# Coder-Yu/SELFRec

Measured on NVIDIA H100. Metric: XSimGCL yelp2018 train steps/sec, higher is better.
Workload: dtype f32

## Files before the change

selfrec_b200/csrc/bpr.cu:

```cuda
#include "common.cuh"

namespace srb {

struct BprArgs {
  const float* emb;
  const float* l2_emb;
  int32_t n_users;
  const int32_t* u_idx;
  const int32_t* i_idx;
  const int32_t* j_idx;
  const int32_t* b_dev;
  int32_t b;
  float emb_scale;
  float reg;
  int32_t l2_terms;
  float l2_div;
  float grad_scale;
  float* losses;
  float* g_emb;
  float* g_l2;
  float* scratch;
};

template <int D>
__device__ __forceinline__ void load_row(const float* base, int row, int lane, float scale, float4 (&r)[(D + 127) / 128]) {
#pragma unroll
  for (int q = 0; q < (D + 127) / 128; ++q) {
    const int c = lane * 4 + q * 128;
    r[q] = (c < D) ? f4_scale(scale, ldg4(base + (size_t)row * D + c)) : f4_zero();
  }
}

template <int D>
__global__ void __launch_bounds__(256) bpr_reduce_kernel(const BprArgs a) {
  constexpr int Q = (D + 127) / 128;
  const int lane = threadIdx.x & 31;
  const int wib = threadIdx.x >> 5;
  const int t = blockIdx.x * (blockDim.x >> 5) + wib;
  const int b = a.b_dev ? min(*a.b_dev, a.b) : a.b;
  float bpr = 0.f, su = 0.f, sp = 0.f, sn = 0.f;
  if (t < b) {
    const int u = a.u_idx[t], p = a.n_users + a.i_idx[t], n = a.n_users + a.j_idx[t];
    float4 ru[Q], rp[Q], rn[Q];
    load_row<D>(a.emb, u, lane, a.emb_scale, ru);
    load_row<D>(a.emb, p, lane, a.emb_scale, rp);
    load_row<D>(a.emb, n, lane, a.emb_scale, rn);
    float pos = 0.f, neg = 0.f;
#pragma unroll
    for (int q = 0; q < Q; ++q) {
      pos += f4_dot(ru[q], rp[q]);
      neg += f4_dot(ru[q], rn[q]);
    }
    pos = warp_sum(pos);
    neg = warp_sum(neg);
    if (a.l2_emb != a.emb) {
      load_row<D>(a.l2_emb, u, lane, 1.f, ru);
      load_row<D>(a.l2_emb, p, lane, 1.f, rp);
      load_row<D>(a.l2_emb, n, lane, 1.f, rn);
    }
#pragma unroll
    for (int q = 0; q < Q; ++q) {
      su += f4_dot(ru[q], ru[q]);
      sp += f4_dot(rp[q], rp[q]);
      sn += f4_dot(rn[q], rn[q]);
    }
    su = warp_sum(su);
    sp = warp_sum(sp);
    sn = warp_sum(sn);
    const float x = pos - neg;
    const float sig = 1.f / (1.f + expf(-x));
    bpr = -logf(1e-5f + sig);
  }
  __shared__ float red[8][4];
  if (lane == 0) {
    red[wib][0] = bpr;
    red[wib][1] = su;
    red[wib][2] = sp;
    red[wib][3] = sn;
  }
  __syncthreads();
  if (threadIdx.x < 4) {
    float s = 0.f;
    for (int w = 0; w < (int)(blockDim.x >> 5); ++w) s += red[w][threadIdx.x];
    atomicAdd(a.scratch + threadIdx.x, s);
  }
}

template <int D>
__global__ void __launch_bounds__(256) bpr_grad_kernel(const BprArgs a) {
  constexpr int Q = (D + 127) / 128;
  const int lane = threadIdx.x & 31;
  const int t = blockIdx.x * (blockDim.x >> 5) + (threadIdx.x >> 5);
  const int b = a.b_dev ? min(*a.b_dev, a.b) : a.b;
  const float fb = (float)b;
  const float nu = sqrtf(a.scratch[1]), np = sqrtf(a.scratch[2]), nn = sqrtf(a.scratch[3]);
  if (blockIdx.x == 0 && threadIdx.x == 0) {
    a.losses[0] = (b > 0) ? a.scratch[0] / fb : 0.f;
    float l2 = nu + np + (a.l2_terms >= 3 ? nn : 0.f);
    a.losses[1] = (b > 0) ? a.reg * (l2 / fb) / a.l2_div : 0.f;
  }
  if (t >= b) return;
  const int u = a.u_idx[t], p = a.n_users + a.i_idx[t], n = a.n_users + a.j_idx[t];
  float4 ru[Q], rp[Q], rn[Q];
  load_row<D>(a.emb, u, lane, a.emb_scale, ru);
  load_row<D>(a.emb, p, lane, a.emb_scale, rp);
  load_row<D>(a.emb, n, lane, a.emb_scale, rn);
  float pos = 0.f, neg = 0.f;
#pragma unroll
  for (int q = 0; q < Q; ++q) {
    pos += f4_dot(ru[q], rp[q]);
    neg += f4_dot(ru[q], rn[q]);
  }
  pos = warp_sum(pos);
  neg = warp_sum(neg);
  const float x = pos - neg;
  const float sig = 1.f / (1.f + expf(-x));
  const float c = a.grad_scale * (-(sig * (1.f - sig)) / (1e-5f + sig)) / fb;
  const float k2 = a.grad_scale * a.reg / (fb * a.l2_div);
  const float ku = nu > 0.f ? k2 / nu : 0.f;
  const float kp = np > 0.f ? k2 / np : 0.f;
  const float kn = (a.l2_terms >= 3 && nn > 0.f) ? k2 / nn : 0.f;
  const bool l2_sep = (a.g_l2 != nullptr);
  float4 lu[Q], lp[Q], ln[Q];
  if (a.l2_emb != a.emb) {
    load_row<D>(a.l2_emb, u, lane, 1.f, lu);
    load_row<D>(a.l2_emb, p, lane, 1.f, lp);
    load_row<D>(a.l2_emb, n, lane, 1.f, ln);
  } else {
#pragma unroll
    for (int q = 0; q < Q; ++q) lu[q] = ru[q], lp[q] = rp[q], ln[q] = rn[q];
  }
  const size_t plane = (size_t)a.b * D;
#pragma unroll
  for (int q = 0; q < Q; ++q) {
    const int col = lane * 4 + q * 128;
    if (col >= D) continue;
    float4 gu = make_float4(c * (rp[q].x - rn[q].x), c * (rp[q].y - rn[q].y), c * (rp[q].z - rn[q].z), c * (rp[q].w - rn[q].w));
    float4 gp = f4_scale(c, ru[q]);
    float4 gn = f4_scale(-c, ru[q]);
    const float4 l2u = f4_scale(ku, lu[q]), l2p = f4_scale(kp, lp[q]), l2n = f4_scale(kn, ln[q]);
    const size_t o = (size_t)t * D + col;
    if (l2_sep) {
      st4(a.g_l2 + o, l2u);
      st4(a.g_l2 + plane + o, l2p);
      st4(a.g_l2 + 2 * plane + o, l2n);
    } else {
      gu = f4_add(gu, l2u);
      gp = f4_add(gp, l2p);
      gn = f4_add(gn, l2n);
    }
    st4(a.g_emb + o, gu);
    st4(a.g_emb + plane + o, gp);
    st4(a.g_emb + 2 * plane + o, gn);
  }
}

template <int D>
__global__ void __launch_bounds__(256) scatter_add_rows_kernel(float* dst, const ScatterSegs segs) {
  const ScatterSeg& sg = segs.s[blockIdx.y];
  const int lane = threadIdx.x & 31;
  const int r = blockIdx.x * (blockDim.x >> 5) + (threadIdx.x >> 5);
  const int nn = sg.n_dev ? min(*sg.n_dev, sg.n) : sg.n;
  if (r >= nn) return;
  int row = sg.rows[r] + sg.row_off;
  if (sg.row_hi > sg.row_lo) {
    if (row < sg.row_lo || row >= sg.row_hi) return;
    row -= sg.row_lo;
  } else if (sg.mod > 0) {
    if (row % sg.mod != sg.rem) return;
    row /= sg.mod;
  }
  for (int c = lane * 4; c < D; c += 128) {
    const float4 v = f4_scale(sg.scale, ldg4(sg.src + (size_t)r * D + c));
    atomicAdd(reinterpret_cast<float4*>(dst + (size_t)row * D + c), v);
  }
}

int scatter_segments(float* dst, int d, const ScatterSegs& segs, cudaStream_t st) {
  if (segs.count == 0) return SRB_OK;
  int max_n = 0;
  for (int q = 0; q < segs.count; ++q) max_n = segs.s[q].n > max_n ? segs.s[q].n : max_n;
  if (max_n == 0) return SRB_OK;
  dim3 grid((max_n + 7) / 8, segs.count);
  switch (d) {
    case 32: scatter_add_rows_kernel<32><<<grid, 256, 0, st>>>(dst, segs); break;
    case 64: scatter_add_rows_kernel<64><<<grid, 256, 0, st>>>(dst, segs); break;
    case 128: scatter_add_rows_kernel<128><<<grid, 256, 0, st>>>(dst, segs); break;
    default: set_error("scatter: unsupported d=%d (32, 64, 128)", d); return SRB_ERR_ARG;
  }
  return post_launch("scatter_add_rows_kernel");
}

struct L2Args {
  int n_terms;
  const float* x[4];
  float* g[4];
  long long n[4];
  int rows[4];
};

__global__ void __launch_bounds__(256) l2_sumsq_kernel(const L2Args a, float* sumsq) {
  const int t = blockIdx.y;
  const long long n = a.n[t];
  float acc = 0.f;
  for (long long i = (long long)blockIdx.x * blockDim.x + threadIdx.x; i < n; i += (long long)gridDim.x * blockDim.x) {
    const float v = a.x[t][i];
    acc = fmaf(v, v, acc);
  }
  acc = warp_sum(acc);
  __shared__ float red[8];
  if ((threadIdx.x & 31) == 0) red[threadIdx.x >> 5] = acc;
  __syncthreads();
  if (threadIdx.x == 0) {
    float s = 0.f;
    for (int w = 0; w < (int)(blockDim.x >> 5); ++w) s += red[w];
    atomicAdd(sumsq + t, s);
  }
}

__global__ void l2_loss_kernel(const L2Args a, const float* sumsq, float reg, float* loss) {
  float l = 0.f;
  for (int t = 0; t < a.n_terms; ++t) l += sqrtf(sumsq[t]) / (float)a.rows[t];
  *loss = l * reg;
}

__global__ void __launch_bounds__(256) l2_grad_kernel(const L2Args a, const float* sumsq, float reg, const float* gout) {
  const int t = blockIdx.y;
  const long long n = a.n[t];
  const float nrm = sqrtf(sumsq[t]);
  const float k = (nrm > 0.f) ? (*gout) * reg / ((float)a.rows[t] * nrm) : 0.f;
  for (long long i = (long long)blockIdx.x * blockDim.x + threadIdx.x; i < n; i += (long long)gridDim.x * blockDim.x)
    a.g[t][i] = k * a.x[t][i];
}

__global__ void adam_prepare_kernel(int32_t* step, float* scalars, double lr, double b1, double b2) {
  const int t = *step + 1;
  *step = t;
  const double bc1 = 1.0 - pow(b1, (double)t);
  const double bc2 = 1.0 - pow(b2, (double)t);
  scalars[0] = (float)(lr / bc1);
  scalars[1] = (float)sqrt(bc2);
}

__global__ void __launch_bounds__(256) adam_step_kernel(float* __restrict__ p, float* __restrict__ m, float* __restrict__ v,
                                                        const float* __restrict__ g, long long n4, long long n,
                                                        const float* __restrict__ scal, float w1, float b2, float w2, float eps) {
  const float step_size = scal[0], bc2_sqrt = scal[1];
  const long long stride = (long long)gridDim.x * blockDim.x;
  for (long long i = (long long)blockIdx.x * blockDim.x + threadIdx.x; i < n4; i += stride) {
    float4 pp = reinterpret_cast<float4*>(p)[i], mm = reinterpret_cast<float4*>(m)[i], vv = reinterpret_cast<float4*>(v)[i];
    const float4 gg = reinterpret_cast<const float4*>(g)[i];
#define SRB_ADAM1(F)                          \
  mm.F = mm.F + w1 * (gg.F - mm.F);           \
  vv.F = vv.F * b2;                           \
  vv.F = vv.F + (w2 * gg.F) * gg.F;           \
  pp.F = pp.F - step_size * (mm.F / (sqrtf(vv.F) / bc2_sqrt + eps));
    SRB_ADAM1(x) SRB_ADAM1(y) SRB_ADAM1(z) SRB_ADAM1(w)
#undef SRB_ADAM1
    reinterpret_cast<float4*>(p)[i] = pp;
    reinterpret_cast<float4*>(m)[i] = mm;
    reinterpret_cast<float4*>(v)[i] = vv;
  }
  for (long long i = n4 * 4 + (long long)blockIdx.x * blockDim.x + threadIdx.x; i < n; i += stride) {
    float mm = m[i], vv = v[i];
    const float gg = g[i];
    mm = mm + w1 * (gg - mm);
    vv = vv * b2;
    vv = vv + (w2 * gg) * gg;
    p[i] = p[i] - step_size * (mm / (sqrtf(vv) / bc2_sqrt + eps));
    m[i] = mm;
    v[i] = vv;
  }
}

}

extern "C" int srb_bpr_l2_fwd_bwd(const srb_bpr_desc* d, void* stream) {
  SRB_REQUIRE(d != nullptr, "bpr: null desc");
  SRB_REQUIRE(d->emb && d->u_idx && d->i_idx && d->j_idx && d->losses && d->g_emb && d->scratch, "bpr: null pointer");
  SRB_REQUIRE(d->l2_terms == 2 || d->l2_terms == 3, "bpr: l2_terms must be 2 or 3");
  SRB_REQUIRE(d->b >= 0, "bpr: negative batch");
  SRB_REQUIRE(d->l2_div > 0.f, "bpr: l2_div must be positive");
  srb::BprArgs a;
  a.emb = d->emb;
  a.l2_emb = d->l2_emb ? d->l2_emb : d->emb;
  SRB_REQUIRE(a.l2_emb == a.emb || d->g_l2, "bpr: a separate l2 table needs g_l2");
  a.n_users = d->n_users;
  a.u_idx = d->u_idx;
  a.i_idx = d->i_idx;
  a.j_idx = d->j_idx;
  a.b_dev = d->b_dev;
  a.b = d->b;
  a.emb_scale = d->emb_scale;
  a.reg = d->reg;
  a.l2_terms = d->l2_terms;
  a.l2_div = d->l2_div;
  a.grad_scale = d->grad_scale;
  a.losses = d->losses;
  a.g_emb = d->g_emb;
  a.g_l2 = d->g_l2;
  a.scratch = d->scratch;
  cudaStream_t st = (cudaStream_t)stream;
  SRB_TRY(srb::check_cuda(cudaMemsetAsync(d->scratch, 0, 8 * sizeof(float), st), "bpr memset"));
  const int blocks = d->b > 0 ? (d->b + 7) / 8 : 1;
  switch (d->d) {
#define SRB_CASE(DD)                                               \
  case DD:                                                         \
    srb::bpr_reduce_kernel<DD><<<blocks, 256, 0, st>>>(a);         \
    SRB_TRY(srb::post_launch("bpr_reduce_kernel"));                \
    srb::bpr_grad_kernel<DD><<<blocks, 256, 0, st>>>(a);           \
    return srb::post_launch("bpr_grad_kernel");
    SRB_CASE(32)
    SRB_CASE(64)
    SRB_CASE(128)
#undef SRB_CASE
    default: srb::set_error("bpr: unsupported d=%d (32, 64, 128)", d->d); return SRB_ERR_ARG;
  }
}

extern "C" int srb_scatter_add_rows(float* dst, int32_t d, const float* src, const int32_t* rows, int32_t n,
                                    const int32_t* n_dev, int32_t row_off, float scale, void* stream) {
  SRB_REQUIRE(dst && src && rows, "scatter: null pointer");
  SRB_REQUIRE(n >= 0, "scatter: negative n");
  srb::ScatterSegs segs;
  segs.count = 1;
  segs.s[0] = {src, rows, n_dev, n, row_off, scale, 0, 0};
  return srb::scatter_segments(dst, d, segs, (cudaStream_t)stream);
}

extern "C" int srb_scatter_add_segments(float* dst, int32_t d, int32_t n_segs, const srb_scatter_seg* in, void* stream) {
  SRB_REQUIRE(dst && in, "scatter: null pointer");
  SRB_REQUIRE(n_segs >= 0 && n_segs <= 8, "scatter: 0..8 segments per launch");
  srb::ScatterSegs segs;
  segs.count = n_segs;
  for (int q = 0; q < n_segs; ++q) {
    SRB_REQUIRE(in[q].src && in[q].rows && in[q].n >= 0, "scatter: bad segment %d", q);
    segs.s[q] = {in[q].src, in[q].rows, in[q].n_dev, in[q].n, in[q].row_off, in[q].scale, 0, 0};
  }
  return srb::scatter_segments(dst, d, segs, (cudaStream_t)stream);
}

extern "C" int srb_adam_prepare(int32_t* step_dev, float* scalars_dev, double lr, double beta1, double beta2, void* stream) {
  SRB_REQUIRE(step_dev && scalars_dev, "adam_prepare: null pointer");
  srb::adam_prepare_kernel<<<1, 1, 0, (cudaStream_t)stream>>>(step_dev, scalars_dev, lr, beta1, beta2);
  return srb::post_launch("adam_prepare_kernel");
}

extern "C" int srb_adam_step(float* p, float* m, float* v, const float* g, int64_t n, const float* scalars_dev, double beta1,
                             double beta2, float eps, void* stream) {
  SRB_REQUIRE(p && m && v && g && scalars_dev, "adam_step: null pointer");
  SRB_REQUIRE(n >= 0, "adam_step: negative n");
  if (n == 0) return SRB_OK;
  const long long n4 = (((uintptr_t)p | (uintptr_t)m | (uintptr_t)v | (uintptr_t)g) & 15) ? 0 : n / 4;
  long long blocks = (n4 + 255) / 256;
  const long long cap = (long long)srb::sm_count() * 8;
  if (blocks > cap) blocks = cap;
  if (blocks < 1) blocks = 1;
  srb::adam_step_kernel<<<(int)blocks, 256, 0, (cudaStream_t)stream>>>(p, m, v, g, n4, n, scalars_dev, (float)(1.0 - beta1), (float)beta2,
                                                                        (float)(1.0 - beta2), eps);
  return srb::post_launch("adam_step_kernel");
}

extern "C" int srb_l2_reg_fwd(int32_t n_terms, const float* const* x, const int64_t* n_elems, const int32_t* rows, float reg,
                              float* sumsq_dev, float* loss_dev, void* stream) {
  SRB_REQUIRE(n_terms >= 1 && n_terms <= 4, "l2_reg: 1..4 terms");
  SRB_REQUIRE(x && n_elems && rows && sumsq_dev && loss_dev, "l2_reg: null pointer");
  srb::L2Args a = {};
  a.n_terms = n_terms;
  long long mx = 1;
  for (int t = 0; t < n_terms; ++t) {
    SRB_REQUIRE(x[t] && rows[t] > 0 && n_elems[t] >= 0, "l2_reg: bad term %d", t);
    a.x[t] = x[t];
    a.n[t] = n_elems[t];
    a.rows[t] = rows[t];
    if (n_elems[t] > mx) mx = n_elems[t];
  }
  cudaStream_t st = (cudaStream_t)stream;
  SRB_TRY(srb::check_cuda(cudaMemsetAsync(sumsq_dev, 0, 4 * sizeof(float), st), "l2 memset"));
  long long bx = (mx + 255) / 256;
  if (bx > 1024) bx = 1024;
  srb::l2_sumsq_kernel<<<dim3((unsigned)bx, n_terms), 256, 0, st>>>(a, sumsq_dev);
  SRB_TRY(srb::post_launch("l2_sumsq_kernel"));
  srb::l2_loss_kernel<<<1, 1, 0, st>>>(a, sumsq_dev, reg, loss_dev);
  return srb::post_launch("l2_loss_kernel");
}

extern "C" int srb_l2_reg_bwd(int32_t n_terms, const float* const* x, float* const* g, const int64_t* n_elems,
                              const int32_t* rows, float reg, const float* sumsq_dev, const float* gout_dev, void* stream) {
  SRB_REQUIRE(n_terms >= 1 && n_terms <= 4, "l2_reg: 1..4 terms");
  SRB_REQUIRE(x && g && n_elems && rows && sumsq_dev && gout_dev, "l2_reg: null pointer");
  srb::L2Args a = {};
  a.n_terms = n_terms;
  long long mx = 1;
  for (int t = 0; t < n_terms; ++t) {
    SRB_REQUIRE(x[t] && g[t] && rows[t] > 0, "l2_reg: bad term %d", t);
    a.x[t] = x[t];
    a.g[t] = g[t];
    a.n[t] = n_elems[t];
    a.rows[t] = rows[t];
    if (n_elems[t] > mx) mx = n_elems[t];
  }
  long long bx = (mx + 255) / 256;
  if (bx > 1024) bx = 1024;
  srb::l2_grad_kernel<<<dim3((unsigned)bx, n_terms), 256, 0, (cudaStream_t)stream>>>(a, sumsq_dev, reg, gout_dev);
  return srb::post_launch("l2_grad_kernel");
}
```

selfrec_b200/csrc/common.cuh:

```cuda
#pragma once
#include <cuda_runtime.h>
#include <stdint.h>
#include <stdio.h>
#include <atomic>
#include "selfrec_b200.h"

#define SRB_FULL_MASK 0xffffffffu

namespace srb {

void set_error(const char* fmt, ...);
extern std::atomic<long long> g_launches;

inline int check_cuda(cudaError_t e, const char* what) {
  if (e != cudaSuccess) {
    set_error("%s: %s", what, cudaGetErrorString(e));
    return SRB_ERR_CUDA;
  }
  return SRB_OK;
}

inline int post_launch(const char* what) {
  g_launches.fetch_add(1, std::memory_order_relaxed);
  return check_cuda(cudaPeekAtLastError(), what);
}

#define SRB_REQUIRE(cond, ...)            \
  do {                                    \
    if (!(cond)) {                        \
      srb::set_error(__VA_ARGS__);        \
      return SRB_ERR_ARG;                 \
    }                                     \
  } while (0)

#define SRB_TRY(expr)                     \
  do {                                    \
    int _rc = (expr);                     \
    if (_rc != SRB_OK) return _rc;        \
  } while (0)

int sm_count();
long long l2_bytes();

struct ScatterSeg {
  const float* src;
  const int32_t* rows;
  const int32_t* n_dev;
  int32_t n;
  int32_t row_off;
  float scale;
  int32_t row_lo, row_hi;
  int32_t mod, rem;
};
struct ScatterSegs {
  int count;
  ScatterSeg s[8];
};
int scatter_segments(float* dst, int d, const ScatterSegs& segs, cudaStream_t st);

__device__ __forceinline__ float warp_sum(float v) {
#pragma unroll
  for (int o = 16; o > 0; o >>= 1) v += __shfl_xor_sync(SRB_FULL_MASK, v, o);
  return v;
}

__device__ __forceinline__ float4 ldg4(const float* p) {
  return __ldg(reinterpret_cast<const float4*>(p));
}

__device__ __forceinline__ void st4(float* p, const float4& v) {
  *reinterpret_cast<float4*>(p) = v;
}

__device__ __forceinline__ float4 f4_zero() { return make_float4(0.f, 0.f, 0.f, 0.f); }

__device__ __forceinline__ float4 f4_fma(float a, const float4& x, const float4& acc) {
  return make_float4(fmaf(a, x.x, acc.x), fmaf(a, x.y, acc.y), fmaf(a, x.z, acc.z),
                     fmaf(a, x.w, acc.w));
}

__device__ __forceinline__ float4 f4_add(const float4& a, const float4& b) {
  return make_float4(a.x + b.x, a.y + b.y, a.z + b.z, a.w + b.w);
}

__device__ __forceinline__ float4 f4_scale(float s, const float4& a) {
  return make_float4(s * a.x, s * a.y, s * a.z, s * a.w);
}

__device__ __forceinline__ float f4_dot(const float4& a, const float4& b) {
  return fmaf(a.w, b.w, fmaf(a.z, b.z, fmaf(a.y, b.y, a.x * b.x)));
}

__device__ __forceinline__ float sgnf(float x) {
  return (x > 0.f) ? 1.f : ((x < 0.f) ? -1.f : 0.f);
}

__device__ __forceinline__ uint4 philox4x32_10(uint4 ctr, uint2 key) {
  const uint32_t M0 = 0xD2511F53u, M1 = 0xCD9E8D57u, W0 = 0x9E3779B9u, W1 = 0xBB67AE85u;
#pragma unroll
  for (int r = 0; r < 10; ++r) {
    uint32_t hi0 = __umulhi(M0, ctr.x), lo0 = M0 * ctr.x;
    uint32_t hi1 = __umulhi(M1, ctr.z), lo1 = M1 * ctr.z;
    ctr = make_uint4(hi1 ^ ctr.y ^ key.x, lo1, hi0 ^ ctr.w ^ key.y, lo0);
    key.x += W0;
    key.y += W1;
  }
  return ctr;
}

__device__ __forceinline__ float u32_to_unit(uint32_t x) {
  return (float)(x >> 8) * (1.0f / 16777216.0f);
}

}
```

selfrec_b200/csrc/engine.cu:

```cuda
#include <mutex>
#include "common.cuh"

namespace srb {

struct Ws {
  float* final_;
  float* cl;
  float* v2;
  float* work0;
  float* work1;
  float* acc0;
  float* acc1;
  float* gd;
  float* rsum;
  float* g_emb;
  float* g_l2;
  float* g_nce;
  float* bpr_scratch;
  float* bpr_losses;
  float* nce_losses;
  int32_t* idx_cat;
  int32_t* n_cat;
  int32_t* batch_rows;
  int32_t* n_hub;
  uint32_t* row_mask;
  int32_t* hub_first;
  int32_t* hub_work;
  float* hub_part;
  int32_t hub_cap;
  void* nce_ws;
  int64_t nce_ws_bytes;
};

static int64_t al(int64_t x) { return (x + 255) / 256 * 256; }

static int64_t carve(const srb_step_desc* s, Ws* w, char* base) {
  const int64_t N = (int64_t)s->n_users + s->n_items, d = s->d, B = s->batch_cap;
  const int64_t nd = al(N * d * 4);
  int64_t off = 0;
  auto take = [&](int64_t bytes) {
    char* p = base ? base + off : nullptr;
    off += al(bytes);
    return p;
  };
  const bool graph = s->model != SRB_MODEL_MF;
  const bool two_views = s->model == SRB_MODEL_SIMGCL || s->model == SRB_MODEL_SGL;
  const bool has_cl = s->model == SRB_MODEL_XSIMGCL || two_views;
  float* f_final = (float*)take(graph ? nd : 0);
  float* f_cl = (float*)take(has_cl ? nd : 0);
  float* f_v2 = (float*)take(two_views ? nd : 0);
  float* f_w0 = (float*)take(graph ? nd : 0);
  float* f_w1 = (float*)take(graph ? nd : 0);
  float* f_a0 = (float*)take(nd);
  float* f_a1 = (float*)take(graph ? nd : 0);
  float* f_gd = (float*)take(graph ? nd : 0);
  float* f_rsum = (float*)take(graph ? nd : 0);
  float* f_gemb = (float*)take(3 * B * d * 4);
  float* f_gl2 = (float*)take(3 * B * d * 4);
  float* f_gnce = (float*)take(has_cl ? 4 * 2 * B * d * 4 : 0);
  float* f_bs = (float*)take(8 * 4);
  float* f_bl = (float*)take(2 * 4);
  float* f_nl = (float*)take(4 * 4);
  int32_t* i_cat = (int32_t*)take(2 * B * 4);
  int32_t* i_ncat = (int32_t*)take(4);
  int32_t* i_brows = (int32_t*)take(4 * 3 * B * 4);
  int32_t* i_nhub = (int32_t*)take(graph ? 32 + ((N + 31) / 32) * 4 : 32);
  uint32_t* u_mask = (uint32_t*)(i_nhub + 8);
  const int64_t hub_cap = graph ? s->adj.hub.n_work : 0;
  int32_t* i_hfirst = (int32_t*)take(hub_cap ? 3 * B * 4 : 0);
  int32_t* i_hwork = (int32_t*)take(hub_cap * 2 * 4);
  float* f_hpart = (float*)take(hub_cap * d * 4);
  const int64_t nws = has_cl ? srb_infonce_workspace_bytes((int32_t)(2 * B), (int32_t)d, 2) : 0;
  void* v_nws = take(nws);
  if (w) {
    w->final_ = f_final;
    w->cl = f_cl;
    w->v2 = f_v2;
    w->work0 = f_w0;
    w->work1 = f_w1;
    w->acc0 = f_a0;
    w->acc1 = f_a1;
    w->gd = f_gd;
    w->rsum = f_rsum;
    w->g_emb = f_gemb;
    w->g_l2 = f_gl2;
    w->g_nce = f_gnce;
    w->bpr_scratch = f_bs;
    w->bpr_losses = f_bl;
    w->nce_losses = f_nl;
    w->idx_cat = i_cat;
    w->n_cat = i_ncat;
    w->batch_rows = i_brows;
    w->n_hub = i_nhub;
    w->row_mask = u_mask;
    w->hub_first = i_hfirst;
    w->hub_work = i_hwork;
    w->hub_part = f_hpart;
    w->hub_cap = (int32_t)hub_cap;
    w->nce_ws = v_nws;
    w->nce_ws_bytes = nws;
  }
  return off;
}

__global__ void build_cat_idx_kernel(const int32_t* batch, int cap, int n_users, int32_t* idx_cat, int32_t* n_cat) {
  const int nu = min(batch[1], cap), ni = min(batch[2], cap);
  const int32_t* uu = batch + SRB_BATCH_HEADER + 3 * cap;
  const int32_t* ui = uu + cap;
  for (int t = blockIdx.x * blockDim.x + threadIdx.x; t < nu + ni; t += gridDim.x * blockDim.x)
    idx_cat[t] = (t < nu) ? uu[t] : n_users + ui[t - nu];
  if (blockIdx.x == 0 && threadIdx.x == 0) *n_cat = nu + ni;
}

__global__ void __launch_bounds__(256) build_batch_rows_kernel(const int32_t* batch, int cap, int n_users, const int32_t* rowptr,
                                                               int row_begin, int n_local, int32_t* rows, int32_t* counters,
                                                               uint32_t* row_mask, int32_t* hub_first, int32_t* hub_work,
                                                               int hub_cap) {
  const int t = blockIdx.x * blockDim.x + threadIdx.x;
  const int b = min(batch[0], cap);
  const int sec = t / cap, k = t % cap;
  if (sec >= 3 || k >= b) return;
  const int32_t* u = batch + SRB_BATCH_HEADER;
  const int grow = (sec == 0) ? u[k] : n_users + u[sec * cap + k];
  const uint32_t bit = 1u << (grow & 31);
  if (atomicOr(row_mask + (grow >> 5), bit) & bit) return;
  const int row = grow - row_begin;
  if (row < 0 || row >= n_local) return;
  const int deg = rowptr[row + 1] - rowptr[row];
  const int cls = (hub_first && deg >= SRB_HUB_MIN_NNZ) ? 0 : (deg >= 128 ? 1 : 2);
  const unsigned mine = __match_any_sync(__activemask(), cls);
  const int lane = threadIdx.x & 31;
  const int leader = __ffs(mine) - 1;
  int base = 0;
  if (lane == leader) base = atomicAdd(counters + cls, __popc(mine));
  base = __shfl_sync(mine, base, leader);
  const int slot = base + __popc(mine & ((1u << lane) - 1));
  rows[cls * 3 * cap + slot] = row;
  if (cls == 0) {
    const int nch = (deg + SRB_HUB_CHUNK - 1) / SRB_HUB_CHUNK;
    const int first = atomicAdd(counters + 4, nch);
    hub_first[slot] = first;
    for (int c = 0; c < nch && first + c < hub_cap; ++c) {
      hub_work[2 * (first + c)] = row;
      hub_work[2 * (first + c) + 1] = c;
    }
  }
}

__global__ void finalize_losses_kernel(const float* bpr_losses, const float* nce_losses, int n_nce, float cl_rate, float* out) {
  float cl = 0.f;
  for (int q = 0; q < n_nce; ++q) cl += nce_losses[q];
  cl *= cl_rate;
  out[0] = bpr_losses[0];
  out[1] = bpr_losses[1];
  out[2] = cl;
  out[3] = bpr_losses[0] + bpr_losses[1] + cl;
}

struct Chain {
  const srb_graph_csr* adj;
  ScatterSegs final_segs;
  ScatterSegs cl_segs;
  ScatterSegs ego_segs;
  int layer_cl;
  bool include_ego;
};

static int spmm_simple(const srb_step_desc* s, const srb_graph_csr* g, const float* x, float* y, const float* extra,
                       bool adam, cudaStream_t st, const uint32_t* col_mask = nullptr) {
  srb_spmm_desc p = {};
  p.col_mask = col_mask;
  p.rowptr = g->rowptr;
  p.colidx = g->colidx;
  p.vals = g->vals;
  p.row_order = g->row_order;
  p.n_long_rows = g->n_long_rows;
  p.n_vlong_rows = g->n_vlong_rows;
  p.hub = g->hub;
  p.n_rows = p.n_cols = s->n_users + s->n_items;
  p.d = s->d;
  p.X = x;
  p.Y = y;
  p.extra = extra;
  p.extra_scale = 1.f;
  if (adam) {
    p.adam_p = s->params;
    p.adam_m = s->adam_m;
    p.adam_v = s->adam_v;
    p.adam_scalars = s->scalars;
    p.beta1 = s->beta1;
    p.beta2 = s->beta2;
    p.adam_eps = s->adam_eps;
  }
  return srb_spmm_csr(&p, st);
}

struct ForkRes {
  cudaStream_t side;
  cudaEvent_t fork, join;
  bool ok;
};
static ForkRes* fork_res(const srb_step_desc* s, ForkRes* own) {
  if (s->fork_stream && s->fork_event && s->join_event) {
    own->side = (cudaStream_t)s->fork_stream;
    own->fork = (cudaEvent_t)s->fork_event;
    own->join = (cudaEvent_t)s->join_event;
    own->ok = true;
    return own;
  }
  static ForkRes res[64] = {};
  static std::mutex mu;
  int dev = 0;
  if (cudaGetDevice(&dev) != cudaSuccess || dev < 0 || dev >= 64) return nullptr;
  std::lock_guard<std::mutex> lock(mu);
  ForkRes& r = res[dev];
  if (!r.ok) {
    if (cudaStreamCreateWithFlags(&r.side, cudaStreamNonBlocking) != cudaSuccess) return nullptr;
    if (cudaEventCreateWithFlags(&r.fork, cudaEventDisableTiming) != cudaSuccess) return nullptr;
    if (cudaEventCreateWithFlags(&r.join, cudaEventDisableTiming) != cudaSuccess) return nullptr;
    r.ok = true;
  }
  return &r;
}

static ScatterSegs merged(const ScatterSegs& a, const ScatterSegs* b) {
  ScatterSegs m = a;
  if (b)
    for (int q = 0; q < b->count && m.count < 8; ++q) m.s[m.count++] = b->s[q];
  return m;
}

static int run_chain(const srb_step_desc* s, const Ws& w, const Chain& c, bool* gd_live, bool last, cudaStream_t st) {
  const int L = s->n_layers, d = s->d;
  const size_t bytes = (size_t)(s->n_users + s->n_items) * d * 4;
  SRB_TRY(check_cuda(cudaMemsetAsync(w.acc0, 0, bytes, st), "chain memset"));
  SRB_TRY(scatter_segments(w.acc0, d, merged(c.final_segs, c.layer_cl == L ? &c.cl_segs : nullptr), st));
  float* x = w.acc0;
  for (int k = L - 1; k >= 1; --k) {
    float* y = (x == w.acc0) ? w.acc1 : w.acc0;
    SRB_TRY(spmm_simple(s, c.adj, x, y, nullptr, false, st, k == L - 1 ? w.row_mask : nullptr));
    SRB_TRY(scatter_segments(y, d, merged(c.final_segs, c.layer_cl == k ? &c.cl_segs : nullptr), st));
    x = y;
  }
  const bool ego_add = (c.include_ego && c.final_segs.count) || c.ego_segs.count;
  if (ego_add && !*gd_live) {
    SRB_TRY(check_cuda(cudaMemsetAsync(w.gd, 0, bytes, st), "chain memset gd"));
    *gd_live = true;
  }
  if (ego_add) {
    if (c.include_ego) SRB_TRY(scatter_segments(w.gd, d, merged(c.final_segs, &c.ego_segs), st));
    else SRB_TRY(scatter_segments(w.gd, d, c.ego_segs, st));
  }
  const float* extra = *gd_live ? w.gd : nullptr;
  const uint32_t* mask = (L == 1) ? w.row_mask : nullptr;
  if (last) return spmm_simple(s, c.adj, x, nullptr, extra, true, st, mask);
  SRB_TRY(spmm_simple(s, c.adj, x, w.gd, extra, false, st, mask));
  *gd_live = true;
  return SRB_OK;
}

static ScatterSeg seg(const float* src, const int32_t* rows, const int32_t* n_dev, int n, int row_off, float scale) {
  ScatterSeg g = {src, rows, n_dev, n, row_off, scale, 0, 0};
  return g;
}

static int encoder(const srb_step_desc* s, const Ws& w, const srb_graph_csr* g, bool include_ego, int noise_mode, int view,
                   int layer_cl, float* final_out, float* cl_out, cudaStream_t st, const float* x1 = nullptr) {
  srb_encoder_desc e = {};
  e.rowptr = g->rowptr;
  e.colidx = g->colidx;
  e.vals = g->vals;
  e.row_order = g->row_order;
  e.n_long_rows = g->n_long_rows;
  e.n_vlong_rows = g->n_vlong_rows;
  e.hub = g->hub;
  e.n = s->n_users + s->n_items;
  e.d = s->d;
  e.n_layers = s->n_layers;
  e.include_ego = include_ego;
  e.layer_cl = layer_cl;
  e.noise_mode = noise_mode;
  if (noise_mode == 1) e.noise = s->noise + (size_t)view * s->n_layers * e.n * e.d;
  e.eps = s->eps;
  e.philox_seed = s->philox_seed;
  e.philox_offset = ((uint64_t)view << 32) | 0x10u;
  e.philox_step_dev = s->step_dev;
  e.E0 = s->params;
  if (cl_out && layer_cl == s->n_layers) {
    e.final_out = final_out;
  } else {
    e.last_rows = w.batch_rows;
    e.n_last_rows = 3 * s->batch_cap;
    e.last_rows_nv_dev = w.n_hub;
    e.last_rows_hub = srb_hub_split{0, w.hub_cap, w.hub_first, w.hub_work, w.hub_part};
    e.last_rows_out = final_out;
    e.final_out = w.rsum;
  }
  e.cl_out = cl_out;
  e.work0 = w.work0;
  e.work1 = w.work1;
  e.x1 = x1;
  return srb_encoder_forward(&e, st);
}

static int perturb_rows(const srb_step_desc* s, const float* x, float* out, int view, cudaStream_t st) {
  const size_t nd = (size_t)(s->n_users + s->n_items) * s->d;
  srb_spmm_desc p = {};
  p.rowptr = s->adj.rowptr;
  p.colidx = s->adj.colidx;
  p.vals = s->adj.vals;
  p.n_rows = p.n_cols = s->n_users + s->n_items;
  p.d = s->d;
  p.X = x;
  p.Y = out;
  p.extra_scale = 1.f;
  p.sum_scale = 1.f;
  p.noise_mode = s->noise_mode;
  if (s->noise_mode == 1) p.noise = s->noise + (size_t)view * s->n_layers * nd;
  p.eps = s->eps;
  p.philox_seed = s->philox_seed;
  p.philox_offset = ((uint64_t)view << 32) | 0x10u;
  p.philox_step_dev = s->step_dev;
  return srb_spmm_epilogue_rows(&p, st);
}

}

extern "C" int64_t srb_step_workspace_bytes(int32_t model, int32_t n, int32_t d, int32_t batch_cap, int32_t n_hub_work) {
  srb_step_desc s = {};
  s.adj.hub.n_work = n_hub_work > 0 ? n_hub_work : 0;
  s.model = model;
  s.n_users = n;
  s.n_items = 0;
  s.d = d;
  s.batch_cap = batch_cap;
  return srb::carve(&s, nullptr, nullptr);
}

extern "C" int srb_train_step(const srb_step_desc* s, void* stream) {
  using namespace srb;
  SRB_REQUIRE(s != nullptr, "step: null desc");
  SRB_REQUIRE(s->model >= SRB_MODEL_MF && s->model <= SRB_MODEL_SGL, "step: unknown model %d", s->model);
  SRB_REQUIRE(s->d == 32 || s->d == 64 || s->d == 128, "step: unsupported d=%d (32, 64, 128)", s->d);
  SRB_REQUIRE(s->n_users > 0 && s->n_items > 0 && s->batch_cap > 0, "step: bad sizes");
  SRB_REQUIRE(s->params && s->adam_m && s->adam_v && s->step_dev && s->scalars && s->losses && s->batch, "step: null pointer");
  SRB_REQUIRE(s->model == SRB_MODEL_MF || s->n_layers >= 1, "step: graph models need n_layers >= 1");
  SRB_REQUIRE(s->model == SRB_MODEL_MF || (s->adj.rowptr && s->adj.colidx && s->adj.vals), "step: null adjacency");
  const int N = s->n_users + s->n_items;
  const int64_t need = srb_step_workspace_bytes(s->model, N, s->d, s->batch_cap, s->model != SRB_MODEL_MF ? s->adj.hub.n_work : 0);
  SRB_REQUIRE(s->workspace && s->workspace_bytes >= need, "step: workspace too small (%lld < %lld)",
              (long long)s->workspace_bytes, (long long)need);
  SRB_REQUIRE(((uintptr_t)s->workspace & 255) == 0, "step: workspace must be 256-byte aligned");
  Ws w;
  carve(s, &w, (char*)s->workspace);
  cudaStream_t st = (cudaStream_t)stream;
  const int B = s->batch_cap, d = s->d, U = s->n_users, L = s->n_layers;
  const int32_t* hdr = s->batch;
  const int32_t* u_idx = s->batch + SRB_BATCH_HEADER;
  const int32_t* i_idx = u_idx + B;
  const int32_t* j_idx = i_idx + B;
  const int32_t* uq_u = j_idx + B;
  const int32_t* uq_i = uq_u + B;
  const int32_t* b_dev = hdr + 0;
  const int32_t* nu_dev = hdr + 1;
  const int32_t* ni_dev = hdr + 2;

  SRB_TRY(srb_adam_prepare(s->step_dev, s->scalars, s->lr, s->beta1, s->beta2, stream));

  if (s->model != SRB_MODEL_MF) {
    SRB_TRY(check_cuda(cudaMemsetAsync(w.n_hub, 0, 32 + (size_t)((U + s->n_items + 31) / 32) * 4, st), "row mask memset"));
    build_batch_rows_kernel<<<(3 * B + 255) / 256, 256, 0, st>>>(s->batch, B, U, s->adj.rowptr, 0, U + s->n_items, w.batch_rows, w.n_hub,
                                                                   w.row_mask, w.hub_cap ? w.hub_first : nullptr, w.hub_work, w.hub_cap);
    SRB_TRY(post_launch("build_batch_rows_kernel"));
  }
  const float* table = s->params;
  int n_nce = 0;
  switch (s->model) {
    case SRB_MODEL_MF: break;
    case SRB_MODEL_LIGHTGCN:
      SRB_TRY(encoder(s, w, &s->adj, true, 0, 0, 0, w.final_, nullptr, st));
      table = w.final_;
      break;
    case SRB_MODEL_XSIMGCL:
      SRB_REQUIRE(s->noise_mode == 1 || s->noise_mode == 2, "step: XSimGCL needs noise_mode 1 or 2");
      SRB_REQUIRE(s->noise_mode != 1 || s->noise, "step: noise tensor missing");
      SRB_TRY(encoder(s, w, &s->adj, false, s->noise_mode, 0, s->layer_cl, w.final_, w.cl, st));
      table = w.final_;
      break;
    case SRB_MODEL_SIMGCL:
      SRB_REQUIRE(s->noise_mode == 1 || s->noise_mode == 2, "step: SimGCL needs noise_mode 1 or 2");
      SRB_REQUIRE(s->noise_mode != 1 || s->noise, "step: noise tensor missing");
      if (L >= 2) {
        SRB_TRY(spmm_simple(s, &s->adj, s->params, w.acc0, nullptr, false, st));
        SRB_TRY(perturb_rows(s, w.acc0, w.acc1, 0, st));
        SRB_TRY(perturb_rows(s, w.acc0, w.gd, 1, st));
        SRB_TRY(encoder(s, w, &s->adj, false, 0, 0, 0, w.final_, nullptr, st, w.acc0));
        SRB_TRY(encoder(s, w, &s->adj, false, s->noise_mode, 0, 0, w.cl, nullptr, st, w.acc1));
        SRB_TRY(encoder(s, w, &s->adj, false, s->noise_mode, 1, 0, w.v2, nullptr, st, w.gd));
      } else {
        SRB_TRY(encoder(s, w, &s->adj, false, 0, 0, 0, w.final_, nullptr, st));
        SRB_TRY(encoder(s, w, &s->adj, false, s->noise_mode, 0, 0, w.cl, nullptr, st));
        SRB_TRY(encoder(s, w, &s->adj, false, s->noise_mode, 1, 0, w.v2, nullptr, st));
      }
      table = w.final_;
      break;
    case SRB_MODEL_SGL:
      SRB_REQUIRE(s->adj_view[0].rowptr && s->adj_view[1].rowptr, "step: SGL needs two view graphs");
      SRB_TRY(encoder(s, w, &s->adj, true, 0, 0, 0, w.final_, nullptr, st));
      SRB_TRY(encoder(s, w, &s->adj_view[0], true, 0, 0, 0, w.cl, nullptr, st));
      SRB_TRY(encoder(s, w, &s->adj_view[1], true, 0, 0, 0, w.v2, nullptr, st));
      table = w.final_;
      break;
  }

  ForkRes fk_own = {};
  ForkRes* fk = (s->model == SRB_MODEL_XSIMGCL || s->model == SRB_MODEL_SIMGCL || s->model == SRB_MODEL_SGL) ? fork_res(s, &fk_own) : nullptr;
  if (fk) {
    SRB_TRY(check_cuda(cudaEventRecord(fk->fork, st), "fork record"));
    SRB_TRY(check_cuda(cudaStreamWaitEvent(fk->side, fk->fork, 0), "fork wait"));
  }
  {
    srb_bpr_desc p = {};
    p.emb = table;
    p.l2_emb = (s->model == SRB_MODEL_LIGHTGCN) ? s->params : table;
    p.n_users = U;
    p.d = d;
    p.u_idx = u_idx;
    p.i_idx = i_idx;
    p.j_idx = j_idx;
    p.b_dev = b_dev;
    p.b = B;
    p.emb_scale = 1.f;
    p.reg = s->reg;
    p.l2_terms = (s->model == SRB_MODEL_SIMGCL || s->model == SRB_MODEL_XSIMGCL) ? 2 : 3;
    p.l2_div = s->l2_div;
    p.grad_scale = 1.f;
    p.losses = w.bpr_losses;
    p.g_emb = w.g_emb;
    p.g_l2 = (s->model == SRB_MODEL_LIGHTGCN) ? w.g_l2 : nullptr;
    p.scratch = w.bpr_scratch;
    SRB_TRY(srb_bpr_l2_fwd_bwd(&p, fk ? (void*)fk->side : stream));
    if (fk) SRB_TRY(check_cuda(cudaEventRecord(fk->join, fk->side), "join record"));
  }

  const size_t gn = (size_t)2 * B * d;
  float* g1a = w.g_nce;
  float* g2a = w.g_nce + gn;
  float* g1b = w.g_nce + 2 * gn;
  float* g2b = w.g_nce + 3 * gn;
  if (s->model == SRB_MODEL_XSIMGCL || s->model == SRB_MODEL_SIMGCL) {
    srb_infonce_desc q = {};
    q.n_problems = 2;
    q.d = d;
    q.b_cos = 1;
    q.temperature = s->tau;
    const float* t1 = (s->model == SRB_MODEL_XSIMGCL) ? w.final_ : w.cl;
    const float* t2 = (s->model == SRB_MODEL_XSIMGCL) ? w.cl : w.v2;
    q.prob[0] = {t1, t2, 0, 0, 1.f, 1.f, uq_u, nu_dev, B, s->cl_rate, g1a, g2a, w.nce_losses + 0};
    q.prob[1] = {t1, t2, U, U, 1.f, 1.f, uq_i, ni_dev, B, s->cl_rate, g1b, g2b, w.nce_losses + 1};
    q.workspace = w.nce_ws;
    q.workspace_bytes = w.nce_ws_bytes;
    SRB_TRY(srb_infonce_fwd_bwd(&q, stream));
    n_nce = 2;
  } else if (s->model == SRB_MODEL_SGL) {
    build_cat_idx_kernel<<<8, 256, 0, st>>>(s->batch, B, U, w.idx_cat, w.n_cat);
    SRB_TRY(post_launch("build_cat_idx_kernel"));
    srb_infonce_desc q = {};
    q.n_problems = 1;
    q.d = d;
    q.b_cos = 1;
    q.temperature = s->tau;
    q.prob[0] = {w.cl, w.v2, 0, 0, 1.f, 1.f, w.idx_cat, w.n_cat, 2 * B, s->cl_rate, g1a, g2a, w.nce_losses + 0};
    q.workspace = w.nce_ws;
    q.workspace_bytes = w.nce_ws_bytes;
    SRB_TRY(srb_infonce_fwd_bwd(&q, stream));
    n_nce = 1;
  }
  if (fk) SRB_TRY(check_cuda(cudaStreamWaitEvent(st, fk->join, 0), "join wait"));
  finalize_losses_kernel<<<1, 1, 0, st>>>(w.bpr_losses, w.nce_losses, n_nce, s->cl_rate, s->losses);
  SRB_TRY(post_launch("finalize_losses_kernel"));

  const size_t plane = (size_t)B * d;
  if (s->model == SRB_MODEL_MF) {
    const size_t bytes = (size_t)N * d * 4;
    SRB_TRY(check_cuda(cudaMemsetAsync(w.acc0, 0, bytes, st), "mf memset"));
    ScatterSegs sg;
    sg.count = 3;
    sg.s[0] = seg(w.g_emb, u_idx, b_dev, B, 0, 1.f);
    sg.s[1] = seg(w.g_emb + plane, i_idx, b_dev, B, U, 1.f);
    sg.s[2] = seg(w.g_emb + 2 * plane, j_idx, b_dev, B, U, 1.f);
    SRB_TRY(scatter_segments(w.acc0, d, sg, st));
    return srb_adam_step(s->params, s->adam_m, s->adam_v, w.acc0, (int64_t)N * d, s->scalars, s->beta1, s->beta2, s->adam_eps,
                         stream);
  }
  const float cm = 1.f / (float)((s->model == SRB_MODEL_LIGHTGCN || s->model == SRB_MODEL_SGL) ? L + 1 : L);
  bool gd_live = false;
  if (s->model == SRB_MODEL_SGL) {
    for (int v = 0; v < 2; ++v) {
      Chain c = {};
      c.adj = &s->adj_view[v];
      c.include_ego = true;
      c.final_segs.count = 1;
      c.final_segs.s[0] = seg(v == 0 ? g1a : g2a, w.idx_cat, w.n_cat, 2 * B, 0, cm);
      SRB_TRY(run_chain(s, w, c, &gd_live, false, st));
    }
  }
  Chain c = {};
  c.adj = &s->adj;
  c.include_ego = (s->model == SRB_MODEL_LIGHTGCN || s->model == SRB_MODEL_SGL);
  ScatterSegs& f = c.final_segs;
  f.count = 3;
  f.s[0] = seg(w.g_emb, u_idx, b_dev, B, 0, cm);
  f.s[1] = seg(w.g_emb + plane, i_idx, b_dev, B, U, cm);
  f.s[2] = seg(w.g_emb + 2 * plane, j_idx, b_dev, B, U, cm);
  if (s->model == SRB_MODEL_LIGHTGCN) {
    c.ego_segs.count = 3;
    c.ego_segs.s[0] = seg(w.g_l2, u_idx, b_dev, B, 0, 1.f);
    c.ego_segs.s[1] = seg(w.g_l2 + plane, i_idx, b_dev, B, U, 1.f);
    c.ego_segs.s[2] = seg(w.g_l2 + 2 * plane, j_idx, b_dev, B, U, 1.f);
  } else if (s->model == SRB_MODEL_XSIMGCL) {
    f.count = 5;
    f.s[3] = seg(g1a, uq_u, nu_dev, B, 0, cm);
    f.s[4] = seg(g1b, uq_i, ni_dev, B, U, cm);
    ScatterSegs& cs = (s->layer_cl >= 1 && s->layer_cl <= L) ? c.cl_segs : c.ego_segs;
    cs.count = 2;
    cs.s[0] = seg(g2a, uq_u, nu_dev, B, 0, 1.f);
    cs.s[1] = seg(g2b, uq_i, ni_dev, B, U, 1.f);
    c.layer_cl = (s->layer_cl >= 1 && s->layer_cl <= L) ? s->layer_cl : 0;
  } else if (s->model == SRB_MODEL_SIMGCL) {
    f.count = 7;
    f.s[3] = seg(g1a, uq_u, nu_dev, B, 0, cm);
    f.s[4] = seg(g1b, uq_i, ni_dev, B, U, cm);
    f.s[5] = seg(g2a, uq_u, nu_dev, B, 0, cm);
    f.s[6] = seg(g2b, uq_i, ni_dev, B, U, cm);
  }
  return run_chain(s, w, c, &gd_live, true, st);
}
```

selfrec_b200/csrc/infonce.cu:

```cuda
#include <stdlib.h>
#include "common.cuh"
#include "infonce_tc.cuh"

namespace srb {

constexpr int NCE_T = 64;
constexpr int NCE_MAX_SPLITS = 8;

struct NceProblem {
  const float* table1;
  const float* table2;
  int32_t row_off1, row_off2;
  float scale1, scale2;
  const int32_t* idx;
  const int32_t* n_dev;
  int32_t n;
  float weight;
  float* g1;
  float* g2;
  float* loss;
  float* V1;
  float* V2;
  float* V1T;
  float* V2T;
  float* inv1;
  float* inv2;
  float* diag;
  float* part_m;
  float* part_l;
  float* dV1;
  float* dV2;
  float* loss_acc;
  float* lse;
};

struct NceArgs {
  int32_t n_problems;
  int32_t np;
  int32_t splits;
  int32_t b_cos;
  float inv_tau;
  NceProblem p[4];
};

__device__ __forceinline__ float tf32_rna(float x) {
  uint32_t r;
  asm("cvt.rna.tf32.f32 %0, %1;" : "=r"(r) : "f"(x));
  return __uint_as_float(r);
}

__device__ __forceinline__ int nce_n(const NceProblem& p) { return p.n_dev ? min(*p.n_dev, p.n) : p.n; }

template <int D>
__global__ void __launch_bounds__(256) nce_prep_kernel(const NceArgs a) {
  const NceProblem& p = a.p[blockIdx.y];
  const int lane = threadIdx.x & 31;
  const int i = blockIdx.x * (blockDim.x >> 5) + (threadIdx.x >> 5);
  if (i >= a.np) return;
  const int n = nce_n(p);
  if (blockIdx.x == 0 && threadIdx.x == 0) *p.loss_acc = 0.f;
  constexpr int Q = (D + 127) / 128;
  float4 v1[Q], v2[Q];
  float s1 = 0.f, s2 = 0.f, s12 = 0.f;
  if (i < n) {
    const int r = p.idx[i];
#pragma unroll
    for (int q = 0; q < Q; ++q) {
      const int c = lane * 4 + q * 128;
      v1[q] = (c < D) ? f4_scale(p.scale1, ldg4(p.table1 + (size_t)(r + p.row_off1) * D + c)) : f4_zero();
      v2[q] = (c < D) ? f4_scale(p.scale2, ldg4(p.table2 + (size_t)(r + p.row_off2) * D + c)) : f4_zero();
      s1 += f4_dot(v1[q], v1[q]);
      s2 += f4_dot(v2[q], v2[q]);
    }
  } else {
#pragma unroll
    for (int q = 0; q < Q; ++q) v1[q] = f4_zero(), v2[q] = f4_zero();
  }
  s1 = warp_sum(s1);
  s2 = warp_sum(s2);
  float i1 = 1.f, i2 = 1.f;
  if (a.b_cos) {
    i1 = 1.f / fmaxf(sqrtf(s1), 1e-12f);
    i2 = 1.f / fmaxf(sqrtf(s2), 1e-12f);
  }
#pragma unroll
  for (int q = 0; q < Q; ++q) {
    const int c = lane * 4 + q * 128;
    if (a.b_cos) {
      const float n1 = fmaxf(sqrtf(s1), 1e-12f), n2 = fmaxf(sqrtf(s2), 1e-12f);
      v1[q] = make_float4(v1[q].x / n1, v1[q].y / n1, v1[q].z / n1, v1[q].w / n1);
      v2[q] = make_float4(v2[q].x / n2, v2[q].y / n2, v2[q].z / n2, v2[q].w / n2);
    }
    s12 += f4_dot(v1[q], v2[q]);
    if (c < D) {
      st4(p.V1 + (size_t)i * D + c, v1[q]);
      st4(p.V2 + (size_t)i * D + c, v2[q]);
      st4(p.dV1 + (size_t)i * D + c, f4_zero());
      st4(p.dV2 + (size_t)i * D + c, f4_zero());
      p.V1T[(size_t)(c + 0) * a.np + i] = v1[q].x;
      p.V1T[(size_t)(c + 1) * a.np + i] = v1[q].y;
      p.V1T[(size_t)(c + 2) * a.np + i] = v1[q].z;
      p.V1T[(size_t)(c + 3) * a.np + i] = v1[q].w;
      p.V2T[(size_t)(c + 0) * a.np + i] = v2[q].x;
      p.V2T[(size_t)(c + 1) * a.np + i] = v2[q].y;
      p.V2T[(size_t)(c + 2) * a.np + i] = v2[q].z;
      p.V2T[(size_t)(c + 3) * a.np + i] = v2[q].w;
    }
  }
  s12 = warp_sum(s12);
  if (lane == 0) {
    p.inv1[i] = i1;
    p.inv2[i] = i2;
    p.diag[i] = s12 * a.inv_tau;
  }
}

__global__ void __launch_bounds__(256) nce_prep_tc_kernel(const NceArgs a) {
  constexpr int D = 64;
  __shared__ float t1[32][D + 1], t2[32][D + 1];
  const NceProblem& p = a.p[blockIdx.y];
  const int lane = threadIdx.x & 31, warp = threadIdx.x >> 5;
  const int i0 = blockIdx.x * 32;
  const int n = nce_n(p);
  if (blockIdx.x == 0 && threadIdx.x == 0) *p.loss_acc = 0.f;
  const size_t nd = (size_t)a.np * D;
  float* hi = p.dV2 + nd;
  float* lo = hi + 4 * nd;
#pragma unroll 1
  for (int rr = 0; rr < 4; ++rr) {
    const int il = warp * 4 + rr, i = i0 + il;
    const int c = lane * 2;
    float2 v1 = make_float2(0.f, 0.f), v2 = make_float2(0.f, 0.f);
    if (i < n) {
      const int r = p.idx[i];
      v1 = *reinterpret_cast<const float2*>(p.table1 + (size_t)(r + p.row_off1) * D + c);
      v2 = *reinterpret_cast<const float2*>(p.table2 + (size_t)(r + p.row_off2) * D + c);
      v1.x *= p.scale1, v1.y *= p.scale1, v2.x *= p.scale2, v2.y *= p.scale2;
    }
    const float s1 = warp_sum(v1.x * v1.x + v1.y * v1.y);
    const float s2 = warp_sum(v2.x * v2.x + v2.y * v2.y);
    float i1 = 1.f, i2 = 1.f;
    if (a.b_cos) {
      const float n1 = fmaxf(sqrtf(s1), 1e-12f), n2 = fmaxf(sqrtf(s2), 1e-12f);
      i1 = 1.f / n1, i2 = 1.f / n2;
      v1.x /= n1, v1.y /= n1, v2.x /= n2, v2.y /= n2;
    }
    const float s12 = warp_sum(v1.x * v2.x + v1.y * v2.y);
    const size_t o = (size_t)i * D + c;
    *reinterpret_cast<float2*>(p.V1 + o) = v1;
    *reinterpret_cast<float2*>(p.V2 + o) = v2;
    *reinterpret_cast<float2*>(p.dV1 + o) = make_float2(0.f, 0.f);
    *reinterpret_cast<float2*>(p.dV2 + o) = make_float2(0.f, 0.f);
    const float2 h1 = make_float2(tf32_rna(v1.x), tf32_rna(v1.y)), h2 = make_float2(tf32_rna(v2.x), tf32_rna(v2.y));
    *reinterpret_cast<float2*>(hi + o) = h1;
    *reinterpret_cast<float2*>(hi + nd + o) = h2;
    *reinterpret_cast<float2*>(lo + o) = make_float2(v1.x - h1.x, v1.y - h1.y);
    *reinterpret_cast<float2*>(lo + nd + o) = make_float2(v2.x - h2.x, v2.y - h2.y);
    t1[il][c] = v1.x, t1[il][c + 1] = v1.y;
    t2[il][c] = v2.x, t2[il][c + 1] = v2.y;
    if (lane == 0) {
      p.inv1[i] = i1;
      p.inv2[i] = i2;
      p.diag[i] = s12 * a.inv_tau;
      p.part_l[i] = 0.f;
    }
  }
  __syncthreads();
  for (int e = threadIdx.x; e < D * 32; e += 256) {
    const int dc = e >> 5, il = e & 31;
    const size_t o = (size_t)dc * a.np + i0 + nce_tperm(il);
    const float x1 = t1[il][dc], x2 = t2[il][dc];
    const float g1 = tf32_rna(x1), g2 = tf32_rna(x2);
    hi[2 * nd + o] = g1;
    hi[3 * nd + o] = g2;
    lo[2 * nd + o] = x1 - g1;
    lo[3 * nd + o] = x2 - g2;
  }
}

template <int D>
__device__ __forceinline__ void load_kmajor(float (*dst)[NCE_T], const float* T, int np, int col0) {
  for (int e = threadIdx.x; e < D * (NCE_T / 4); e += blockDim.x) {
    const int k = e / (NCE_T / 4), c4 = e % (NCE_T / 4);
    *reinterpret_cast<float4*>(&dst[k][c4 * 4]) = *reinterpret_cast<const float4*>(T + (size_t)k * np + col0 + c4 * 4);
  }
}

template <int D>
__device__ __forceinline__ void load_rowmajor(float (*dst)[D], const float* V, int row0) {
  for (int e = threadIdx.x; e < NCE_T * (D / 4); e += blockDim.x) {
    const int r = e / (D / 4), c4 = e % (D / 4);
    *reinterpret_cast<float4*>(&dst[r][c4 * 4]) = *reinterpret_cast<const float4*>(V + (size_t)(row0 + r) * D + c4 * 4);
  }
}

template <int D>
__device__ __forceinline__ void s_tile(const float (*AsT)[NCE_T], const float (*BsT)[NCE_T], int ty, int tx, float (&s)[4][4]) {
#pragma unroll
  for (int r = 0; r < 4; ++r)
#pragma unroll
    for (int c = 0; c < 4; ++c) s[r][c] = 0.f;
#pragma unroll 8
  for (int k = 0; k < D; ++k) {
    const float4 av = *reinterpret_cast<const float4*>(&AsT[k][ty * 4]);
    const float4 bv = *reinterpret_cast<const float4*>(&BsT[k][tx * 4]);
    const float ar[4] = {av.x, av.y, av.z, av.w};
    const float bc[4] = {bv.x, bv.y, bv.z, bv.w};
#pragma unroll
    for (int r = 0; r < 4; ++r)
#pragma unroll
      for (int c = 0; c < 4; ++c) s[r][c] = fmaf(ar[r], bc[c], s[r][c]);
  }
}

template <int D>
struct NceLseSmem {
  float AsT[D][NCE_T];
  float BsT[D][NCE_T];
};

template <int D>
__global__ void __launch_bounds__(256) nce_lse_kernel(const NceArgs a) {
  extern __shared__ __align__(16) unsigned char smem_raw[];
  NceLseSmem<D>& sm = *reinterpret_cast<NceLseSmem<D>*>(smem_raw);
  const NceProblem& p = a.p[blockIdx.z];
  const int n = nce_n(p);
  const int i0 = blockIdx.x * NCE_T;
  if (i0 >= n) return;
  const int split = blockIdx.y;
  const int ty = threadIdx.x >> 4, tx = threadIdx.x & 15;
  load_kmajor<D>(sm.AsT, p.V1T, a.np, i0);
  float m[4], l[4];
#pragma unroll
  for (int r = 0; r < 4; ++r) m[r] = -INFINITY, l[r] = 0.f;
  const int ntiles = (n + NCE_T - 1) / NCE_T;
  const float L2E = 1.4426950408889634f;
  for (int jt = split; jt < ntiles; jt += a.splits) {
    const int j0 = jt * NCE_T;
    __syncthreads();
    load_kmajor<D>(sm.BsT, p.V2T, a.np, j0);
    __syncthreads();
    float s[4][4];
    s_tile<D>(sm.AsT, sm.BsT, ty, tx, s);
#pragma unroll
    for (int r = 0; r < 4; ++r) {
      float tm = -INFINITY;
#pragma unroll
      for (int c = 0; c < 4; ++c) {
        s[r][c] = (j0 + tx * 4 + c < n) ? s[r][c] * a.inv_tau : -INFINITY;
        tm = fmaxf(tm, s[r][c]);
      }
      const float mn = fmaxf(m[r], tm);
      if (mn > -INFINITY) {
        float acc = 0.f;
#pragma unroll
        for (int c = 0; c < 4; ++c) acc += exp2f((s[r][c] - mn) * L2E);
        l[r] = l[r] * exp2f((m[r] - mn) * L2E) + acc;
        m[r] = mn;
      }
    }
  }
#pragma unroll
  for (int r = 0; r < 4; ++r) {
#pragma unroll
    for (int o = 8; o > 0; o >>= 1) {
      const float mo = __shfl_xor_sync(SRB_FULL_MASK, m[r], o);
      const float lo = __shfl_xor_sync(SRB_FULL_MASK, l[r], o);
      const float mn = fmaxf(m[r], mo);
      if (mn > -INFINITY) {
        l[r] = l[r] * exp2f((m[r] - mn) * L2E) + lo * exp2f((mo - mn) * L2E);
        m[r] = mn;
      }
    }
    if (tx == 0) {
      const int i = i0 + ty * 4 + r;
      p.part_m[(size_t)split * a.np + i] = m[r];
      p.part_l[(size_t)split * a.np + i] = l[r];
    }
  }
}

template <int D>
struct NceGradSmem {
  float AsT[D][NCE_T];
  float BsT[D][NCE_T];
  float Ar[NCE_T][D];
  float Br[NCE_T][D];
  float Gs[NCE_T][NCE_T];
  float GsT[NCE_T][NCE_T];
  float lse[NCE_T];
  float red[8];
};

template <int D>
__global__ void __launch_bounds__(256) nce_grad_kernel(const NceArgs a) {
  constexpr int CW = D / 16;
  extern __shared__ __align__(16) unsigned char smem_raw[];
  NceGradSmem<D>& sm = *reinterpret_cast<NceGradSmem<D>*>(smem_raw);
  const NceProblem& p = a.p[blockIdx.z];
  const int n = nce_n(p);
  const int i0 = blockIdx.x * NCE_T;
  if (i0 >= n) return;
  const int split = blockIdx.y;
  const int ty = threadIdx.x >> 4, tx = threadIdx.x & 15;
  const float L2E = 1.4426950408889634f;
  load_kmajor<D>(sm.AsT, p.V1T, a.np, i0);
  load_rowmajor<D>(sm.Ar, p.V1, i0);
  if (threadIdx.x < NCE_T) {
    const int i = i0 + threadIdx.x;
    float M = -INFINITY;
    for (int s = 0; s < a.splits; ++s) M = fmaxf(M, p.part_m[(size_t)s * a.np + i]);
    float Lsum = 0.f;
    for (int s = 0; s < a.splits; ++s) {
      const float ms = p.part_m[(size_t)s * a.np + i];
      if (ms > -INFINITY) Lsum += p.part_l[(size_t)s * a.np + i] * exp2f((ms - M) * L2E);
    }
    const float lse = (i < n) ? M + logf(Lsum) : 0.f;
    sm.lse[threadIdx.x] = lse;
    float contrib = (split == 0 && i < n) ? lse - p.diag[i] : 0.f;
    contrib = warp_sum(contrib);
    if ((threadIdx.x & 31) == 0) sm.red[threadIdx.x >> 5] = contrib;
  }
  __syncthreads();
  if (threadIdx.x == 0 && split == 0) atomicAdd(p.loss_acc, sm.red[0] + sm.red[1]);
  const float gscale = p.weight * a.inv_tau / (float)n;
  float o1[4][CW];
#pragma unroll
  for (int r = 0; r < 4; ++r)
#pragma unroll
    for (int q = 0; q < CW; ++q) o1[r][q] = 0.f;
  const int ntiles = (n + NCE_T - 1) / NCE_T;
  for (int jt = split; jt < ntiles; jt += a.splits) {
    const int j0 = jt * NCE_T;
    __syncthreads();
    load_kmajor<D>(sm.BsT, p.V2T, a.np, j0);
    load_rowmajor<D>(sm.Br, p.V2, j0);
    __syncthreads();
    float s[4][4];
    s_tile<D>(sm.AsT, sm.BsT, ty, tx, s);
#pragma unroll
    for (int r = 0; r < 4; ++r) {
      const int i = i0 + ty * 4 + r;
      const float lse = sm.lse[ty * 4 + r];
#pragma unroll
      for (int c = 0; c < 4; ++c) {
        const int j = j0 + tx * 4 + c;
        float g = 0.f;
        if (i < n && j < n) {
          g = exp2f((s[r][c] * a.inv_tau - lse) * L2E);
          if (i == j) g -= 1.f;
          g *= gscale;
        }
        s[r][c] = g;
      }
      *reinterpret_cast<float4*>(&sm.Gs[ty * 4 + r][tx * 4]) = make_float4(s[r][0], s[r][1], s[r][2], s[r][3]);
    }
#pragma unroll
    for (int c = 0; c < 4; ++c) {
      const int jl = tx * 4 + c;
      *reinterpret_cast<float4*>(&sm.GsT[jl][((ty ^ (jl >> 2)) & 15) * 4]) = make_float4(s[0][c], s[1][c], s[2][c], s[3][c]);
    }
    __syncthreads();
#pragma unroll 4
    for (int j = 0; j < NCE_T; ++j) {
      const float4 av = *reinterpret_cast<const float4*>(&sm.GsT[j][((ty ^ (j >> 2)) & 15) * 4]);
      const float ar[4] = {av.x, av.y, av.z, av.w};
      float bq[CW];
#pragma unroll
      for (int q = 0; q < CW; ++q) bq[q] = sm.Br[j][tx * CW + q];
#pragma unroll
      for (int r = 0; r < 4; ++r)
#pragma unroll
        for (int q = 0; q < CW; ++q) o1[r][q] = fmaf(ar[r], bq[q], o1[r][q]);
    }
    float qv[4][CW];
#pragma unroll
    for (int r = 0; r < 4; ++r)
#pragma unroll
      for (int q = 0; q < CW; ++q) qv[r][q] = 0.f;
#pragma unroll 4
    for (int i = 0; i < NCE_T; ++i) {
      const float4 av = *reinterpret_cast<const float4*>(&sm.Gs[i][ty * 4]);
      const float ar[4] = {av.x, av.y, av.z, av.w};
      float bq[CW];
#pragma unroll
      for (int q = 0; q < CW; ++q) bq[q] = sm.Ar[i][tx * CW + q];
#pragma unroll
      for (int r = 0; r < 4; ++r)
#pragma unroll
        for (int q = 0; q < CW; ++q) qv[r][q] = fmaf(ar[r], bq[q], qv[r][q]);
    }
#pragma unroll
    for (int r = 0; r < 4; ++r) {
      const int j = j0 + ty * 4 + r;
      if (j < n) {
#pragma unroll
        for (int q = 0; q < CW; ++q) atomicAdd(p.dV2 + (size_t)j * D + tx * CW + q, qv[r][q]);
      }
    }
  }
#pragma unroll
  for (int r = 0; r < 4; ++r) {
    const int i = i0 + ty * 4 + r;
    if (i < n) {
#pragma unroll
      for (int q = 0; q < CW; ++q) atomicAdd(p.dV1 + (size_t)i * D + tx * CW + q, o1[r][q]);
    }
  }
}

template <int D>
__global__ void __launch_bounds__(256) nce_finish_kernel(const NceArgs a) {
  const NceProblem& p = a.p[blockIdx.y];
  const int lane = threadIdx.x & 31;
  const int i = blockIdx.x * (blockDim.x >> 5) + (threadIdx.x >> 5);
  const int n = nce_n(p);
  if (blockIdx.x == 0 && threadIdx.x == 0) *p.loss = (n > 0) ? *p.loss_acc / (float)n : 0.f;
  if (i >= n) return;
  constexpr int Q = (D + 127) / 128;
#pragma unroll 1
  for (int side = 0; side < 2; ++side) {
    const float* V = side ? p.V2 : p.V1;
    const float* dV = side ? p.dV2 : p.dV1;
    float* g = side ? p.g2 : p.g1;
    const float inv = side ? p.inv2[i] : p.inv1[i];
    float4 vh[Q], dv[Q];
    float dot = 0.f;
#pragma unroll
    for (int q = 0; q < Q; ++q) {
      const int c = lane * 4 + q * 128;
      vh[q] = (c < D) ? *reinterpret_cast<const float4*>(V + (size_t)i * D + c) : f4_zero();
      dv[q] = (c < D) ? *reinterpret_cast<const float4*>(dV + (size_t)i * D + c) : f4_zero();
      dot += f4_dot(vh[q], dv[q]);
    }
    dot = warp_sum(dot);
#pragma unroll
    for (int q = 0; q < Q; ++q) {
      const int c = lane * 4 + q * 128;
      if (c >= D) continue;
      float4 o = dv[q];
      if (a.b_cos) {
        o = make_float4((dv[q].x - vh[q].x * dot) * inv, (dv[q].y - vh[q].y * dot) * inv, (dv[q].z - vh[q].z * dot) * inv,
                        (dv[q].w - vh[q].w * dot) * inv);
      }
      st4(g + (size_t)i * D + c, o);
    }
  }
}

static inline int64_t align_up(int64_t x, int64_t a) { return (x + a - 1) / a * a; }
static inline int nce_np(int n) { return (int)align_up(n > 0 ? n : 1, 128); }

static int64_t nce_problem_floats(int np, int d) {
  return 14ll * np * d + 4ll * np + 2ll * NCE_MAX_SPLITS * np + 64;
}

__global__ void __launch_bounds__(256) nce_tc_finish_kernel(const NceArgs a) {
  constexpr int D = 64;
  const NceProblem& p = a.p[blockIdx.y];
  const int lane = threadIdx.x & 31;
  const int i = blockIdx.x * (blockDim.x >> 5) + (threadIdx.x >> 5);
  const int n = nce_n(p);
  if (blockIdx.x == 0 && threadIdx.x == 0) *p.loss = (n > 0) ? *p.loss_acc / (float)n : 0.f;
  if (i >= n) return;
  const float li = p.part_l[i];
  const float pii = expf(p.diag[i] - a.inv_tau) / li;
  const float gs = p.weight * a.inv_tau / (float)n;
  const float cd = (pii - 1.f) * gs;
  const float2 v1 = *reinterpret_cast<const float2*>(p.V1 + (size_t)i * D + lane * 2);
  const float2 v2 = *reinterpret_cast<const float2*>(p.V2 + (size_t)i * D + lane * 2);
#pragma unroll 1
  for (int side = 0; side < 2; ++side) {
    const float2 vh = side ? v2 : v1;
    const float2 vo = side ? v1 : v2;
    float2 dv = *reinterpret_cast<const float2*>((side ? p.dV2 : p.dV1) + (size_t)i * D + lane * 2);
    if (side == 0) dv.x *= gs / li, dv.y *= gs / li;
    dv.x = fmaf(cd, vo.x, dv.x);
    dv.y = fmaf(cd, vo.y, dv.y);
    const float dot = warp_sum(vh.x * dv.x + vh.y * dv.y);
    const float inv = side ? p.inv2[i] : p.inv1[i];
    float2 o = dv;
    if (a.b_cos) o = make_float2((dv.x - vh.x * dot) * inv, (dv.y - vh.y * dot) * inv);
    *reinterpret_cast<float2*>((side ? p.g2 : p.g1) + (size_t)i * D + lane * 2) = o;
  }
}

static int nce_impl() {
  static int impl = -1;
  if (impl < 0) {
    const char* e = getenv("SRB_NCE_IMPL");
    impl = e ? atoi(e) : 0;
  }
  return impl;
}

static int nce_launch_tc(const NceArgs& a, int n_problems, cudaStream_t st) {
  const int np = a.np;
  const int d = NT_D;
  {
    dim3 grid(np / 32, n_problems);
    nce_prep_tc_kernel<<<grid, 256, 0, st>>>(a);
    SRB_TRY(post_launch("nce_prep_tc_kernel"));
  }
  NtMaps maps;
  NtArgs t;
  t.np = np;
  t.inv_tau = a.inv_tau;
  const int row_blocks = np / NT_T;
  int splits = sm_count() / (row_blocks * n_problems);
  if (splits < 1) splits = 1;
  if (splits > NT_MAX_SPLITS) splits = NT_MAX_SPLITS;
  if (splits > row_blocks) splits = row_blocks;
  t.splits = splits;
  const long long nd = (long long)np * d;
  for (int q = 0; q < n_problems; ++q) {
    const NceProblem& p = a.p[q];
    float* hi = p.dV2 + nd;
    float* lo = hi + 4 * nd;
    for (int h = 0; h < 2; ++h) {
      float* r = h ? lo : hi;
      SRB_REQUIRE(make_tmap_f32_rows(&maps.v1r[q][h], r, (uint64_t)np, d, NT_T) == 0 &&
                      make_tmap_f32_rows(&maps.v2r[q][h], r + nd, (uint64_t)np, d, NT_T) == 0 &&
                      make_tmap_f32_rows(&maps.v1c[q][h], r, (uint64_t)np, d, NT_C) == 0 &&
                      make_tmap_f32_rows(&maps.v2c[q][h], r + nd, (uint64_t)np, d, NT_C) == 0 &&
                      make_tmap_f32_rows(&maps.v1t[q][h], r + 2 * nd, (uint64_t)d, (uint64_t)np, NT_D) == 0 &&
                      make_tmap_f32_rows(&maps.v2t[q][h], r + 3 * nd, (uint64_t)d, (uint64_t)np, NT_D) == 0,
                  "infonce: cuTensorMapEncodeTiled failed");
    }
    NtProblem& o = t.p[q];
    o.n = p.n;
    o.n_dev = p.n_dev;
    o.weight = p.weight;
    o.diag = p.diag;
    o.lsum = p.part_l;
    o.dV1 = p.dV1;
    o.dV2 = p.dV2;
    o.loss_acc = p.loss_acc;
  }
  for (int q = n_problems; q < 2; ++q) {
    for (int h = 0; h < 2; ++h) {
      maps.v1r[q][h] = maps.v1r[0][h];
      maps.v2r[q][h] = maps.v2r[0][h];
      maps.v1c[q][h] = maps.v1c[0][h];
      maps.v2c[q][h] = maps.v2c[0][h];
      maps.v1t[q][h] = maps.v1t[0][h];
      maps.v2t[q][h] = maps.v2t[0][h];
    }
    t.p[q] = t.p[0];
  }
  const size_t smem = NtSmem::total + 1024;
  static bool attr_done = false;
  if (!attr_done) {
    SRB_TRY(check_cuda(cudaFuncSetAttribute(nce_tc_kernel<1>, cudaFuncAttributeMaxDynamicSharedMemorySize, (int)smem), "nce tc attr"));
    SRB_TRY(check_cuda(cudaFuncSetAttribute(nce_tc_kernel<2>, cudaFuncAttributeMaxDynamicSharedMemorySize, (int)smem), "nce tc attr"));
    attr_done = true;
  }
  dim3 grid(row_blocks, splits, n_problems);
  nce_tc_kernel<1><<<grid, NT_THREADS, smem, st>>>(maps, t);
  SRB_TRY(post_launch("nce_tc_kernel<pass_a>"));
  nce_tc_kernel<2><<<grid, NT_THREADS, smem, st>>>(maps, t);
  SRB_TRY(post_launch("nce_tc_kernel<pass_b>"));
  {
    dim3 g2((np + 7) / 8, n_problems);
    nce_tc_finish_kernel<<<g2, 256, 0, st>>>(a);
    SRB_TRY(post_launch("nce_tc_finish_kernel"));
  }
  return SRB_OK;
}

template <int D>
static int nce_launch(const NceArgs& a, int n_problems, cudaStream_t st) {
  const int np = a.np;
  {
    dim3 grid((np + 7) / 8, n_problems);
    nce_prep_kernel<D><<<grid, 256, 0, st>>>(a);
    SRB_TRY(post_launch("nce_prep_kernel"));
  }
  {
    static bool attr_done = false;
    if (!attr_done) {
      SRB_TRY(check_cuda(cudaFuncSetAttribute(nce_lse_kernel<D>, cudaFuncAttributeMaxDynamicSharedMemorySize, (int)sizeof(NceLseSmem<D>)), "nce lse smem attr"));
      SRB_TRY(check_cuda(cudaFuncSetAttribute(nce_grad_kernel<D>, cudaFuncAttributeMaxDynamicSharedMemorySize, (int)sizeof(NceGradSmem<D>)), "nce grad smem attr"));
      attr_done = true;
    }
    dim3 grid(np / NCE_T, a.splits, n_problems);
    nce_lse_kernel<D><<<grid, 256, sizeof(NceLseSmem<D>), st>>>(a);
    SRB_TRY(post_launch("nce_lse_kernel"));
    nce_grad_kernel<D><<<grid, 256, sizeof(NceGradSmem<D>), st>>>(a);
    SRB_TRY(post_launch("nce_grad_kernel"));
  }
  {
    dim3 grid((np + 7) / 8, n_problems);
    nce_finish_kernel<D><<<grid, 256, 0, st>>>(a);
    SRB_TRY(post_launch("nce_finish_kernel"));
  }
  return SRB_OK;
}

}

extern "C" int64_t srb_infonce_workspace_bytes(int32_t max_n, int32_t d, int32_t n_problems) {
  if (max_n < 0 || d <= 0 || n_problems <= 0) return 0;
  return srb::nce_problem_floats(srb::nce_np(max_n), d) * 4 * n_problems;
}

extern "C" int srb_infonce_fwd_bwd(const srb_infonce_desc* d, void* stream) {
  SRB_REQUIRE(d != nullptr, "infonce: null desc");
  SRB_REQUIRE(d->n_problems >= 1 && d->n_problems <= 4, "infonce: n_problems must be 1..4");
  SRB_REQUIRE(d->temperature > 0.f, "infonce: temperature must be positive");
  SRB_REQUIRE(d->d == 32 || d->d == 64 || d->d == 128, "infonce: unsupported d=%d (32, 64, 128)", d->d);
  int max_n = 0;
  for (int q = 0; q < d->n_problems; ++q) {
    const srb_infonce_problem& s = d->prob[q];
    SRB_REQUIRE(s.table1 && s.table2 && s.idx && s.g1 && s.g2 && s.loss, "infonce: null pointer in problem %d", q);
    SRB_REQUIRE(s.n >= 0, "infonce: negative n");
    if (s.n > max_n) max_n = s.n;
  }
  SRB_REQUIRE(d->workspace && d->workspace_bytes >= srb_infonce_workspace_bytes(max_n, d->d, d->n_problems),
              "infonce: workspace too small (%lld < %lld)", (long long)d->workspace_bytes,
              (long long)srb_infonce_workspace_bytes(max_n, d->d, d->n_problems));
  if (max_n == 0) {
    for (int q = 0; q < d->n_problems; ++q)
      SRB_TRY(srb::check_cuda(cudaMemsetAsync(d->prob[q].loss, 0, 4, (cudaStream_t)stream), "infonce memset"));
    return SRB_OK;
  }
  srb::NceArgs a;
  a.n_problems = d->n_problems;
  a.np = srb::nce_np(max_n);
  a.b_cos = d->b_cos;
  a.inv_tau = 1.0f / d->temperature;
  const int row_blocks = a.np / srb::NCE_T;
  int splits = (2 * srb::sm_count() + row_blocks * d->n_problems - 1) / (row_blocks * d->n_problems);
  if (splits < 1) splits = 1;
  if (splits > srb::NCE_MAX_SPLITS) splits = srb::NCE_MAX_SPLITS;
  if (splits > row_blocks) splits = row_blocks;
  a.splits = splits;
  float* w = reinterpret_cast<float*>(d->workspace);
  const int64_t per = srb::nce_problem_floats(a.np, d->d);
  for (int q = 0; q < d->n_problems; ++q) {
    const srb_infonce_problem& s = d->prob[q];
    srb::NceProblem& p = a.p[q];
    p.table1 = s.table1;
    p.table2 = s.table2;
    p.row_off1 = s.row_off1;
    p.row_off2 = s.row_off2;
    p.scale1 = s.scale1;
    p.scale2 = s.scale2;
    p.idx = s.idx;
    p.n_dev = s.n_dev;
    p.n = s.n;
    p.weight = s.weight;
    p.g1 = s.g1;
    p.g2 = s.g2;
    p.loss = s.loss;
    float* base = w + per * q;
    const int64_t nd = (int64_t)a.np * d->d;
    p.V1 = base;
    p.V2 = base + nd;
    p.V1T = base + 2 * nd;
    p.V2T = base + 3 * nd;
    p.dV1 = base + 4 * nd;
    p.dV2 = base + 5 * nd;
    float* t = base + 14 * nd;
    p.inv1 = t;
    p.inv2 = t + a.np;
    p.diag = t + 2 * a.np;
    p.part_m = t + 3 * a.np;
    p.part_l = t + 3 * a.np + (int64_t)srb::NCE_MAX_SPLITS * a.np;
    p.lse = t + 3 * a.np + 2ll * srb::NCE_MAX_SPLITS * a.np;
    p.loss_acc = p.lse + a.np;
  }
  cudaStream_t st = (cudaStream_t)stream;
  const int impl = srb::nce_impl();
  if (d->d == 64 && d->b_cos && impl != 1 && d->n_problems <= 2 && a.inv_tau <= 40.f) return srb::nce_launch_tc(a, d->n_problems, st);
  SRB_REQUIRE(impl != 2, "infonce: SRB_NCE_IMPL=2 (tensor cores) needs d == 64, b_cos and temperature >= 0.025");
  switch (d->d) {
    case 32: return srb::nce_launch<32>(a, d->n_problems, st);
    case 64: return srb::nce_launch<64>(a, d->n_problems, st);
    default: return srb::nce_launch<128>(a, d->n_problems, st);
  }
}
```

selfrec_b200/csrc/infonce_tc.cuh:

```cuda
#pragma once
#include "common.cuh"
#include "tc_common.cuh"

namespace srb {

using namespace tc;

constexpr int NT_D = 64;
constexpr int NT_T = 128;
constexpr int NT_C = 64;
constexpr int NT_STAGES = 2;
constexpr int NT_THREADS = 256 + 32;
constexpr int NT_MAX_SPLITS = 8;
constexpr uint32_t NT_ATILE = NT_T * NT_D * 4;
constexpr uint32_t NT_BTILE = NT_C * NT_D * 4;
constexpr uint32_t NT_TTILE = NT_D * NT_C * 4;
constexpr uint32_t NT_STAGE = 2 * NT_BTILE + 2 * NT_TTILE;

__host__ __device__ __forceinline__ int nce_tperm(int i) { return (i & ~7) | (((i & 7) >> 1) + 4 * (i & 1)); }

struct NtSmem {
  static constexpr uint32_t a_off = 0;
  static constexpr uint32_t b_off = a_off + 2 * NT_ATILE;
  static constexpr uint32_t bar_off = b_off + NT_STAGES * NT_STAGE;
  static constexpr uint32_t total = bar_off + 1024;
};

struct NtProblem {
  int32_t n;
  const int32_t* n_dev;
  float weight;
  const float* diag;
  float* lsum;
  float* dV1;
  float* dV2;
  float* loss_acc;
};

struct NtArgs {
  int32_t np;
  int32_t splits;
  float inv_tau;
  NtProblem p[2];
};

struct NtMaps {
  CUtensorMap v1r[2][2], v2r[2][2], v1c[2][2], v2c[2][2], v1t[2][2], v2t[2][2];
};

__device__ __forceinline__ int nt_n(const NtProblem& p) { return p.n_dev ? min(*p.n_dev, p.n) : p.n; }

__device__ __forceinline__ float to_tf32_rna(float x) {
  uint32_t r;
  asm("cvt.rna.tf32.f32 %0, %1;" : "=r"(r) : "f"(x));
  return __uint_as_float(r);
}

__device__ __forceinline__ float ex2_approx(float x) {
  float y;
  asm("ex2.approx.ftz.f32 %0, %1;" : "=f"(y) : "f"(x));
  return y;
}

template <int MODE>
__global__ void __launch_bounds__(NT_THREADS, 1) nce_tc_kernel(const __grid_constant__ NtMaps maps, const NtArgs a) {
  extern __shared__ __align__(1024) uint8_t nt_smem_raw[];
  uint8_t* sm = reinterpret_cast<uint8_t*>((reinterpret_cast<uintptr_t>(nt_smem_raw) + 1023) & ~(uintptr_t)1023);
  uint64_t* bars = reinterpret_cast<uint64_t*>(sm + NtSmem::bar_off);
  uint64_t* bar_full = bars;
  uint64_t* bar_empty = bars + NT_STAGES;
  uint64_t* bar_a = bars + 2 * NT_STAGES;
  float* colc = reinterpret_cast<float*>(bars + 8);

  const int prob = blockIdx.z;
  const NtProblem& P = a.p[prob];
  const int n = nt_n(P);
  const int r0 = blockIdx.x * NT_T;
  if (r0 >= n) return;
  const int split = blockIdx.y;
  const int warp = threadIdx.x >> 5;
  const int lane = threadIdx.x & 31;
  const int n_tiles = (n + NT_C - 1) / NT_C;
  const int my_tiles = (n_tiles - split + a.splits - 1) / a.splits;
  if (my_tiles <= 0) return;
  const CUtensorMap* map_row = (MODE == 2) ? maps.v2r[prob] : maps.v1r[prob];
  const CUtensorMap* map_col = (MODE == 2) ? maps.v1c[prob] : maps.v2c[prob];
  const CUtensorMap* map_colt = (MODE == 2) ? maps.v1t[prob] : maps.v2t[prob];

  if (threadIdx.x == 0) {
    for (int s = 0; s < NT_STAGES; ++s) {
      mbar_init(bar_full + s, 1);
      mbar_init(bar_empty + s, 2);
    }
    mbar_init(bar_a, 1);
    fence_barrier_init();
  }
  __syncthreads();

  if (warp == 8) {
    if (elect_one()) {
      mbar_arrive_expect_tx(bar_a, 2 * NT_ATILE);
      for (int h = 0; h < 2; ++h)
        for (int c = 0; c < 2; ++c) tma_load_2d(sm + NtSmem::a_off + h * NT_ATILE + c * 16384, &map_row[h], bar_a, c * 32, r0);
      for (int k = 0; k < my_tiles; ++k) {
        const int t = split + k * a.splits;
        const int s = k % NT_STAGES;
        uint8_t* st = sm + NtSmem::b_off + s * NT_STAGE;
        mbar_wait(bar_empty + s, ((k / NT_STAGES) & 1) ^ 1);
        mbar_arrive_expect_tx(bar_full + s, NT_STAGE);
        for (int h = 0; h < 2; ++h)
          for (int c = 0; c < 2; ++c) {
            tma_load_2d(st + h * NT_BTILE + c * 8192, &map_col[h], bar_full + s, c * 32, t * NT_C);
            tma_load_2d(st + 2 * NT_BTILE + h * NT_TTILE + c * 8192, &map_colt[h], bar_full + s, t * NT_C + c * 32, 0);
          }
      }
    }
    return;
  }
  const int wg = warp >> 2;
  const int w4 = warp & 3, g = lane >> 2, tq = lane & 3;
  const int et = threadIdx.x;
  const int row_a = r0 + wg * 64 + w4 * 16 + g;
  const float L2E = 1.4426950408889634f;
  const float sc = a.inv_tau * L2E;
  const float gscale = P.weight * a.inv_tau / (float)n;
  const float lg = log2f(gscale);
  float l_run[2] = {0.f, 0.f};
  auto col_const = [&](int col) -> float {
    float off = -INFINITY, contrib = 0.f;
    if (col < n) {
      const float lse = a.inv_tau + logf(P.lsum[col]);
      off = lg - lse * L2E;
      contrib = lse - P.diag[col];
    }
    if (blockIdx.x == 0) {
      contrib = warp_sum(contrib);
      if (lane == 0) atomicAdd(P.loss_acc, contrib);
    }
    return off;
  };
  float next_colc = 0.f;
  if (MODE == 2) {
    if (et < NT_C) colc[et] = col_const(split * NT_C + et);
    named_bar_sync(1, 256);
  }
  const uint32_t a_base = smem_u32(sm + NtSmem::a_off + wg * 8192);
  float d[32];
#pragma unroll
  for (int j = 0; j < 32; ++j) d[j] = 0.f;
  mbar_wait(bar_a, 0);
  for (int k = 0; k < my_tiles; ++k) {
    const int t = split + k * a.splits;
    const int s = k % NT_STAGES;
    const int cb = t * NT_C;
    if (MODE == 2 && et < NT_C && k + 1 < my_tiles) next_colc = col_const((t + a.splits) * NT_C + et);
    mbar_wait(bar_full + s, (k / NT_STAGES) & 1);
    const uint32_t b_base = smem_u32(sm + NtSmem::b_off + s * NT_STAGE);
    float sv[32];
    wgmma_fence();
#pragma unroll
    for (int pr = 0; pr < 3; ++pr) {
      const uint32_t ab = a_base + (pr == 2 ? NT_ATILE : 0);
      const uint32_t bb = b_base + (pr == 1 ? NT_BTILE : 0);
#pragma unroll
      for (int c = 0; c < 2; ++c)
#pragma unroll
        for (int kk = 0; kk < 4; ++kk)
          wgmma_m64n64k8_tf32_ss(sv, make_smem_desc_k_sw128(ab + c * 16384 + kk * 32), make_smem_desc_k_sw128(bb + c * 8192 + kk * 32),
                                 (pr | c | kk) ? 1u : 0u);
    }
    wgmma_commit();
    wgmma_wait<0>();
    uint32_t hi[32], lo[32];
    const float* cc = colc + (k & 1) * NT_C;
#pragma unroll
    for (int j = 0; j < 32; ++j) {
      const int cl = 8 * (j >> 2) + 2 * tq + (j & 1);
      const int rh = (j >> 1) & 1;
      const float off = (MODE == 1) ? -sc : cc[cl];
      float x = ex2_approx(fmaf(sv[j], sc, off));
      if (MODE == 1) {
        x = (cb + cl < n) ? x : 0.f;
        l_run[rh] += x;
      }
      x = (cb + cl == row_a + 8 * rh) ? 0.f : x;
      const float h = to_tf32_rna(x);
      hi[j] = __float_as_uint(h);
      lo[j] = __float_as_uint(x - h);
    }
    const uint32_t bt_base = b_base + 2 * NT_BTILE;
    wgmma_fence();
#pragma unroll
    for (int pr = 0; pr < 3; ++pr) {
      const uint32_t (&ga)[32] = (pr == 1) ? lo : hi;
      const uint32_t vb = bt_base + (pr == 2 ? NT_TTILE : 0);
#pragma unroll
      for (int kk = 0; kk < 8; ++kk)
        wgmma_m64n64k8_tf32_rs(d, ga[4 * kk], ga[4 * kk + 2], ga[4 * kk + 1], ga[4 * kk + 3],
                               make_smem_desc_k_sw128(vb + (kk >> 2) * 8192 + (kk & 3) * 32), 1u);
    }
    wgmma_commit();
    wgmma_wait<0>();
    if ((threadIdx.x & 127) == 0) mbar_arrive(bar_empty + s);
    if (MODE == 2) {
      if (et < NT_C && k + 1 < my_tiles) colc[((k + 1) & 1) * NT_C + et] = next_colc;
      named_bar_sync(1, 256);
    }
  }
#pragma unroll
  for (int rh = 0; rh < 2; ++rh) {
    const int row = row_a + 8 * rh;
    if (MODE == 1) {
      float l = l_run[rh];
      l += __shfl_xor_sync(SRB_FULL_MASK, l, 1);
      l += __shfl_xor_sync(SRB_FULL_MASK, l, 2);
      if (tq == 0 && row < n) atomicAdd(P.lsum + row, l);
    }
    if (row < n) {
      float* out = ((MODE == 1) ? P.dV1 : P.dV2) + (size_t)row * NT_D;
#pragma unroll
      for (int cg = 0; cg < 8; ++cg)
        atomicAdd(reinterpret_cast<float2*>(out + 8 * cg + 2 * tq), make_float2(d[4 * cg + 2 * rh], d[4 * cg + 2 * rh + 1]));
    }
  }
}

}
```

selfrec_b200/csrc/spmm.cu:

```cuda
#include <stdlib.h>
#include "spmm_args.cuh"

namespace srb {

__device__ __forceinline__ void st4_cs(float* p, const float4& v, int stream) {
  if (stream) __stcs(reinterpret_cast<float4*>(p), v);
  else st4(p, v);
}

__device__ __forceinline__ void st4_peer(float* p, const float4& v, int mc) {
  if (mc) asm volatile("multimem.st.weak.global.v4.f32 [%0], {%1, %2, %3, %4};" ::"l"(p), "f"(v.x), "f"(v.y), "f"(v.z), "f"(v.w) : "memory");
  else st4(p, v);
}

template <int D>
__device__ __forceinline__ void spmm_epilogue(const SpmmArgs& a, int row, int gl, float4 acc0, float4 acc1, bool valid) {
  constexpr int LPR = D / 8;
  constexpr int HALF = D / 2;
  {
    if (a.stage_peer[0]) {
      if (!valid) return;
      int o = 0;
#pragma unroll 1
      while (row >= a.stage_bounds[o + 1]) ++o;
      float* dst = a.stage_peer[o] + ((size_t)a.stage_rank * a.stage_cap + (row - a.stage_bounds[o])) * D + gl * 4;
      st4(dst, acc0);
      st4(dst + HALF, acc1);
      return;
    }
    const size_t off = (size_t)(a.row_begin + row) * D + gl * 4;
    float4 y0 = acc0, y1 = acc1;
    if (a.extra && valid) {
      y0 = f4_fma(a.extra_scale, *reinterpret_cast<const float4*>(a.extra + off), y0);
      y1 = f4_fma(a.extra_scale, *reinterpret_cast<const float4*>(a.extra + off + HALF), y1);
    }
    if (a.noise_mode) {
      float4 n0 = f4_zero(), n1 = f4_zero();
      if (a.noise_mode == 1) {
        if (valid) {
          n0 = ldg4(a.noise + off);
          n1 = ldg4(a.noise + off + HALF);
        }
      } else {
        const uint32_t stp = a.pstep ? (uint32_t)*a.pstep : 0u;
        const uint32_t grow = (uint32_t)(a.noise_row_base + (a.row_begin + row) * a.noise_row_stride);
        const uint32_t vw = a.poff.y << 16;
        const uint4 r0 = philox4x32_10(make_uint4(grow, (uint32_t)gl | vw, a.poff.x, stp), a.pkey);
        const uint4 r1 = philox4x32_10(make_uint4(grow, (uint32_t)(gl + LPR) | vw, a.poff.x, stp), a.pkey);
        n0 = make_float4(u32_to_unit(r0.x), u32_to_unit(r0.y), u32_to_unit(r0.z), u32_to_unit(r0.w));
        n1 = make_float4(u32_to_unit(r1.x), u32_to_unit(r1.y), u32_to_unit(r1.z), u32_to_unit(r1.w));
      }
      float ss = f4_dot(n0, n0) + f4_dot(n1, n1);
#pragma unroll
      for (int o = LPR / 2; o > 0; o >>= 1) ss += __shfl_xor_sync(SRB_FULL_MASK, ss, o);
      const float nrm = fmaxf(sqrtf(ss), 1e-12f);
#define SRB_PERT(Y, N, F) Y.F += sgnf(Y.F) * (N.F / nrm) * a.eps;
      SRB_PERT(y0, n0, x) SRB_PERT(y0, n0, y) SRB_PERT(y0, n0, z) SRB_PERT(y0, n0, w)
      SRB_PERT(y1, n1, x) SRB_PERT(y1, n1, y) SRB_PERT(y1, n1, z) SRB_PERT(y1, n1, w)
#undef SRB_PERT
    }
    if (!valid) return;
    if (a.Y) {
      st4_cs(a.Y + off, y0, a.stream);
      st4_cs(a.Y + off + HALF, y1, a.stream);
    }
    if (a.world > 0 && a.peer[0]) {
#pragma unroll 1
      for (int g = 0; g < a.world; ++g) {
        st4_peer(a.peer[g] + off, y0, a.peer_mc);
        st4_peer(a.peer[g] + off + HALF, y1, a.peer_mc);
      }
    }
    if (a.sum_out) {
      float4 s0 = y0, s1 = y1;
      if (a.sum_in) {
        s0 = f4_add(s0, *reinterpret_cast<const float4*>(a.sum_in + off));
        s1 = f4_add(s1, *reinterpret_cast<const float4*>(a.sum_in + off + HALF));
      }
      s0 = f4_scale(a.sum_scale, s0);
      s1 = f4_scale(a.sum_scale, s1);
      st4_cs(a.sum_out + off, s0, a.stream);
      st4_cs(a.sum_out + off + HALF, s1, a.stream);
      if (a.world > 0 && a.peer_sum[0]) {
#pragma unroll 1
        for (int g = 0; g < a.world; ++g) {
          st4_peer(a.peer_sum[g] + off, s0, a.peer_mc);
          st4_peer(a.peer_sum[g] + off + HALF, s1, a.peer_mc);
        }
      }
    }
    if (a.ap) {
      const float step_size = a.ascal[0];
      const float bc2_sqrt = a.ascal[1];
#pragma unroll
      for (int h = 0; h < 2; ++h) {
        const size_t o2 = off + h * HALF;
        const float4 g = h ? y1 : y0;
        float4 p4 = *reinterpret_cast<const float4*>(a.ap + o2);
        float4 m = *reinterpret_cast<const float4*>(a.am + o2);
        float4 v4 = *reinterpret_cast<const float4*>(a.av + o2);
#define SRB_ADAM1(F)                                          \
  m.F = m.F + a.w1 * (g.F - m.F);                             \
  v4.F = v4.F * a.b2;                                         \
  v4.F = v4.F + (a.w2 * g.F) * g.F;                           \
  p4.F = p4.F - step_size * (m.F / (sqrtf(v4.F) / bc2_sqrt + a.aeps));
        SRB_ADAM1(x) SRB_ADAM1(y) SRB_ADAM1(z) SRB_ADAM1(w)
#undef SRB_ADAM1
        st4(a.ap + o2, p4);
        st4_cs(a.am + o2, m, a.stream);
        st4_cs(a.av + o2, v4, a.stream);
        if (a.world > 0 && a.peer_p[0]) {
#pragma unroll 1
          for (int g = 0; g < a.world; ++g) st4_peer(a.peer_p[g] + o2, p4, a.peer_mc);
        }
      }
    }
  }
}

__device__ __forceinline__ void cp_async16(void* smem_dst, const void* gsrc) {
  const uint32_t s = (uint32_t)__cvta_generic_to_shared(smem_dst);
  asm volatile("cp.async.ca.shared.global [%0], [%1], 16;" ::"r"(s), "l"(gsrc) : "memory");
}
__device__ __forceinline__ void cp_async_commit() { asm volatile("cp.async.commit_group;" ::: "memory"); }
__device__ __forceinline__ void cp_async_wait_all() { asm volatile("cp.async.wait_group 0;" ::: "memory"); }

constexpr int SPMM_STAGE_F4 = 8 * 32;

template <int D, bool MASKED, bool ASYNC = false>
__device__ __forceinline__ void spmm_gather(const SpmmArgs& a, int p, int end, int stride, int gl, float4& acc0, float4& acc1,
                                            float4* stg = nullptr) {
  constexpr int LPR = D / 8;
  constexpr int HALF = D / 2;
  constexpr int SB = LPR < 4 ? LPR : 4;
  constexpr bool masked = MASKED;
  const int lane = threadIdx.x & 31;
  const int gbase = lane - gl;
  int c = 0;
  float v = 0.f;
  bool hit = false;
  if (p + gl < end) {
    c = a.stream ? __ldcs(a.colidx + p + gl) : __ldg(a.colidx + p + gl);
    v = a.stream ? __ldcs(a.vals + p + gl) : __ldg(a.vals + p + gl);
    if (masked) hit = (__ldg(a.col_mask + (c >> 5)) >> (c & 31)) & 1u;
  }
  while (__any_sync(SRB_FULL_MASK, p < end)) {
    int cn = 0;
    float vn = 0.f;
    bool hitn = false;
    if (p + stride + gl < end) {
      cn = a.stream ? __ldcs(a.colidx + p + stride + gl) : __ldg(a.colidx + p + stride + gl);
      vn = a.stream ? __ldcs(a.vals + p + stride + gl) : __ldg(a.vals + p + stride + gl);
      if (masked) hitn = (__ldg(a.col_mask + (cn >> 5)) >> (cn & 31)) & 1u;
    }
    if (!masked && ASYNC && LPR >= 2 * SB) {
#pragma unroll
      for (int j0 = 0; j0 < LPR; j0 += 2 * SB) {
        if (j0 > 0 && !__any_sync(SRB_FULL_MASK, p + j0 < end)) break;
        float vb[SB];
#pragma unroll
        for (int j = 0; j < SB; ++j) {
          const int cc = __shfl_sync(SRB_FULL_MASK, c, j0 + SB + j, LPR);
          vb[j] = __shfl_sync(SRB_FULL_MASK, v, j0 + SB + j, LPR);
          const float* xr = a.X + (size_t)cc * D + gl * 4;
          cp_async16(stg + (2 * j) * 32, xr);
          cp_async16(stg + (2 * j + 1) * 32, xr + HALF);
        }
        cp_async_commit();
        float vv[SB];
        float4 x0[SB], x1[SB];
#pragma unroll
        for (int j = 0; j < SB; ++j) {
          const int cc = __shfl_sync(SRB_FULL_MASK, c, j0 + j, LPR);
          vv[j] = __shfl_sync(SRB_FULL_MASK, v, j0 + j, LPR);
          const float* xr = a.X + (size_t)cc * D + gl * 4;
          x0[j] = ldg4(xr);
          x1[j] = ldg4(xr + HALF);
        }
#pragma unroll
        for (int j = 0; j < SB; ++j) {
          acc0 = f4_fma(vv[j], x0[j], acc0);
          acc1 = f4_fma(vv[j], x1[j], acc1);
        }
        cp_async_wait_all();
#pragma unroll
        for (int j = 0; j < SB; ++j) {
          acc0 = f4_fma(vb[j], stg[(2 * j) * 32], acc0);
          acc1 = f4_fma(vb[j], stg[(2 * j + 1) * 32], acc1);
        }
      }
    } else if (!masked) {
#pragma unroll
      for (int j0 = 0; j0 < LPR; j0 += SB) {
        if (j0 > 0 && !__any_sync(SRB_FULL_MASK, p + j0 < end)) break;
        float vv[SB];
        float4 x0[SB], x1[SB];
#pragma unroll
        for (int j = 0; j < SB; ++j) {
          const int cc = __shfl_sync(SRB_FULL_MASK, c, j0 + j, LPR);
          vv[j] = __shfl_sync(SRB_FULL_MASK, v, j0 + j, LPR);
          const float* xr = a.X + (size_t)cc * D + gl * 4;
          x0[j] = ldg4(xr);
          x1[j] = ldg4(xr + HALF);
        }
#pragma unroll
        for (int j = 0; j < SB; ++j) {
          acc0 = f4_fma(vv[j], x0[j], acc0);
          acc1 = f4_fma(vv[j], x1[j], acc1);
        }
      }
    } else {
      uint32_t gm = (__ballot_sync(SRB_FULL_MASK, hit) >> gbase) & ((1u << LPR) - 1u);
      while (__any_sync(SRB_FULL_MASK, gm != 0)) {
        float vv[SB];
        float4 x0[SB], x1[SB];
#pragma unroll
        for (int j = 0; j < SB; ++j) {
          const int src = gm ? (__ffs(gm) - 1) : 0;
          const bool live = gm != 0;
          gm &= gm - 1;
          const int cc = __shfl_sync(SRB_FULL_MASK, c, gbase + src);
          const float vs = __shfl_sync(SRB_FULL_MASK, v, gbase + src);
          vv[j] = live ? vs : 0.f;
          const float* xr = a.X + (size_t)(live ? cc : 0) * D + gl * 4;
          x0[j] = ldg4(xr);
          x1[j] = ldg4(xr + HALF);
        }
#pragma unroll
        for (int j = 0; j < SB; ++j) {
          acc0 = f4_fma(vv[j], x0[j], acc0);
          acc1 = f4_fma(vv[j], x1[j], acc1);
        }
      }
    }
    c = cn;
    v = vn;
    hit = hitn;
    p += stride;
  }
}

__device__ __forceinline__ void xor_reduce_groups(float4& acc0, float4& acc1, int lpr) {
  for (int o = lpr; o < 32; o <<= 1) {
    acc0.x += __shfl_xor_sync(SRB_FULL_MASK, acc0.x, o);
    acc0.y += __shfl_xor_sync(SRB_FULL_MASK, acc0.y, o);
    acc0.z += __shfl_xor_sync(SRB_FULL_MASK, acc0.z, o);
    acc0.w += __shfl_xor_sync(SRB_FULL_MASK, acc0.w, o);
    acc1.x += __shfl_xor_sync(SRB_FULL_MASK, acc1.x, o);
    acc1.y += __shfl_xor_sync(SRB_FULL_MASK, acc1.y, o);
    acc1.z += __shfl_xor_sync(SRB_FULL_MASK, acc1.z, o);
    acc1.w += __shfl_xor_sync(SRB_FULL_MASK, acc1.w, o);
  }
}

template <int D, bool MASKED, bool ASYNC>
__global__ void __launch_bounds__(256) spmm_hub_kernel(const SpmmArgs a) {
  constexpr int LPR = D / 8;
  const int lane = threadIdx.x & 31;
  const int wib = threadIdx.x >> 5;
  __shared__ float4 stage[ASYNC ? 8 * SPMM_STAGE_F4 : 1];
  float4* stg = ASYNC ? stage + wib * SPMM_STAGE_F4 + lane : nullptr;
  const int grp = lane / LPR;
  const int gl = lane % LPR;
  const int n_work = a.seg ? a.n_cta : (a.n_vlong_dev ? min(a.n_vlong_dev[4], a.n_work) : a.n_work);
  __shared__ float4 part[8][2][LPR];
  for (int k = blockIdx.x; k < n_work; k += gridDim.x) {
    int w = k, beg, end;
    if (a.seg) {
      w = __ldg(a.order_cta + k);
      beg = __ldg(a.seg + 2 * w);
      end = __ldg(a.seg + 2 * w + 1);
    } else {
      const int row = __ldg(a.hub_work + 2 * w);
      const int ci = __ldg(a.hub_work + 2 * w + 1);
      const int rbeg = __ldg(a.rowptr + row), rend = __ldg(a.rowptr + row + 1);
      beg = min(rend, rbeg + ci * SRB_HUB_CHUNK);
      end = min(rend, beg + SRB_HUB_CHUNK);
    }
    const int per = ((end - beg + 255) / 256) * 32;
    const int wbeg = beg + wib * per;
    const int wend = min(end, wbeg + per);
    float4 acc0 = f4_zero(), acc1 = f4_zero();
    spmm_gather<D, MASKED, ASYNC>(a, wbeg + grp * LPR, wend, 32, gl, acc0, acc1, stg);
    xor_reduce_groups(acc0, acc1, LPR);
    if (grp == 0) {
      part[wib][0][gl] = acc0;
      part[wib][1][gl] = acc1;
    }
    __syncthreads();
    if (wib == 0 && grp == 0) {
      acc0 = f4_zero();
      acc1 = f4_zero();
#pragma unroll
      for (int q = 0; q < 8; ++q) {
        acc0 = f4_add(acc0, part[q][0][gl]);
        acc1 = f4_add(acc1, part[q][1][gl]);
      }
      float* dst = a.hub_part + (size_t)w * D + gl * 4;
      st4(dst, acc0);
      st4(dst + D / 2, acc1);
    }
    __syncthreads();
  }
}

template <int D, bool MASKED, bool ASYNC>
__global__ void __launch_bounds__(256) spmm_seg_warp_kernel(const SpmmArgs a) {
  constexpr int LPR = D / 8;
  const int lane = threadIdx.x & 31;
  __shared__ float4 stage[ASYNC ? 8 * SPMM_STAGE_F4 : 1];
  float4* stg = ASYNC ? stage + (threadIdx.x >> 5) * SPMM_STAGE_F4 + lane : nullptr;
  const int grp = lane / LPR;
  const int gl = lane % LPR;
  const int warp0 = (blockIdx.x * blockDim.x + threadIdx.x) >> 5;
  const int nwarps = (gridDim.x * blockDim.x) >> 5;
  for (int k = warp0; k < a.n_warp; k += nwarps) {
    const int w = __ldg(a.order_warp + k);
    const int beg = __ldg(a.seg + 2 * w), end = __ldg(a.seg + 2 * w + 1);
    float4 acc0 = f4_zero(), acc1 = f4_zero();
    spmm_gather<D, MASKED, ASYNC>(a, beg + grp * LPR, end, 32, gl, acc0, acc1, stg);
    xor_reduce_groups(acc0, acc1, LPR);
    if (grp == 0) {
      float* dst = a.hub_part + (size_t)w * D + gl * 4;
      st4(dst, acc0);
      st4(dst + D / 2, acc1);
    }
  }
}

template <int D>
__global__ void __launch_bounds__(256) spmm_hub_finish_kernel(const SpmmArgs a) {
  constexpr int LPR = D / 8;
  constexpr int RPW = 32 / LPR;
  const int lane = threadIdx.x & 31;
  const int grp = lane / LPR;
  const int gl = lane % LPR;
  const int warp0 = (blockIdx.x * blockDim.x + threadIdx.x) >> 5;
  const int nwarps = (gridDim.x * blockDim.x) >> 5;
  const int n_huge = a.n_vlong_dev ? min(a.n_vlong_dev[0], a.n_rows) : a.n_huge;
  peer_wait(a.ps);
  for (int vr = warp0; vr < n_huge; vr += nwarps) {
    const int row = __ldg(a.row_order + vr);
    const int first = __ldg(a.hub_first + vr);
    const int deg = __ldg(a.rowptr + row + 1) - __ldg(a.rowptr + row);
    const int nch = a.seg ? __ldg(a.seg_cnt + vr) : (deg + SRB_HUB_CHUNK - 1) / SRB_HUB_CHUNK;
    float4 acc0 = f4_zero(), acc1 = f4_zero();
    for (int c = grp; c < nch; c += RPW) {
      const float* src = a.hub_part + (size_t)(first + c) * D + gl * 4;
      acc0 = f4_add(acc0, *reinterpret_cast<const float4*>(src));
      acc1 = f4_add(acc1, *reinterpret_cast<const float4*>(src + D / 2));
    }
    xor_reduce_groups(acc0, acc1, LPR);
    spmm_epilogue<D>(a, row, gl, acc0, acc1, grp == 0);
  }
}

template <int D, bool MASKED, bool ASYNC>
__global__ void __launch_bounds__(256) spmm_csr_kernel(const SpmmArgs a) {
  constexpr int LPR = D / 8;
  constexpr int RPW = 32 / LPR;
  const int lane = threadIdx.x & 31;
  const int wib = threadIdx.x >> 5;
  __shared__ float4 stage[ASYNC ? 8 * SPMM_STAGE_F4 : 1];
  float4* stg = ASYNC ? stage + wib * SPMM_STAGE_F4 + lane : nullptr;
  const int grp = lane / LPR;
  const int gl = lane % LPR;
  const int warp0 = (blockIdx.x * blockDim.x + threadIdx.x) >> 5;
  const int nwarps = (gridDim.x * blockDim.x) >> 5;

  peer_wait(a.ps);
  int n_vlong = a.n_vlong, n_long = a.n_long, n_short = a.n_rows - a.n_huge - a.n_vlong - a.n_long;
  const int32_t* ro_v = a.row_order ? a.row_order + a.n_huge : nullptr;
  const int32_t* ro_l = a.row_order ? ro_v + n_vlong : nullptr;
  const int32_t* ro_s = a.row_order ? ro_l + n_long : nullptr;
  int id_l = n_vlong, id_s = n_vlong + n_long;
  if (a.n_vlong_dev) {
    n_vlong = min(a.n_vlong_dev[1], a.n_rows);
    n_long = min(a.n_vlong_dev[2], a.n_rows);
    n_short = min(a.n_vlong_dev[3], a.n_rows);
    ro_v = a.row_order + a.n_rows;
    ro_l = a.row_order + 2 * a.n_rows;
    ro_s = a.row_order + 3 * a.n_rows;
  }
  __shared__ float4 part[8][2][LPR];
  for (int vr = blockIdx.x; vr < n_vlong; vr += gridDim.x) {
    const int row = ro_v ? __ldg(ro_v + vr) : vr;
    const int beg = __ldg(a.rowptr + row);
    const int end = __ldg(a.rowptr + row + 1);
    const int per = ((end - beg + 255) / 256) * 32;
    const int wbeg = beg + wib * per;
    const int wend = min(end, wbeg + per);
    float4 acc0 = f4_zero(), acc1 = f4_zero();
    spmm_gather<D, MASKED, ASYNC>(a, wbeg + grp * LPR, wend, 32, gl, acc0, acc1, stg);
    xor_reduce_groups(acc0, acc1, LPR);
    if (grp == 0) {
      part[wib][0][gl] = acc0;
      part[wib][1][gl] = acc1;
    }
    __syncthreads();
    if (wib == 0) {
      acc0 = f4_zero();
      acc1 = f4_zero();
#pragma unroll
      for (int w = 0; w < 8; ++w) {
        acc0 = f4_add(acc0, part[w][0][gl]);
        acc1 = f4_add(acc1, part[w][1][gl]);
      }
      spmm_epilogue<D>(a, row, gl, acc0, acc1, grp == 0);
    }
    __syncthreads();
  }

  const int n_items = n_long + (n_short + RPW - 1) / RPW;
  for (int item = warp0; item < n_items; item += nwarps) {
    const bool is_long = item < n_long;
    const int k = is_long ? item : (item - n_long) * RPW + grp;
    bool valid = is_long || k < n_short;
    int row = 0, p = 0, end = 0;
    if (valid) {
      if (is_long) row = ro_l ? __ldg(ro_l + k) : id_l + k;
      else row = ro_s ? __ldg(ro_s + k) : id_s + k;
      p = __ldg(a.rowptr + row);
      end = __ldg(a.rowptr + row + 1);
    }
    if (is_long) p += grp * LPR;
    float4 acc0 = f4_zero(), acc1 = f4_zero();
    spmm_gather<D, MASKED, ASYNC>(a, p, end, is_long ? 32 : LPR, gl, acc0, acc1, stg);
    if (is_long) {
      xor_reduce_groups(acc0, acc1, LPR);
      valid = valid && grp == 0;
    }
    spmm_epilogue<D>(a, row, gl, acc0, acc1, valid);
  }
  peer_signal(a.ps);
}

__device__ __forceinline__ float4 multimem_ld_reduce_add4(const float* mc) {
  float4 v;
  asm volatile("multimem.ld_reduce.relaxed.sys.global.add.v4.f32 {%0, %1, %2, %3}, [%4];"
               : "=f"(v.x), "=f"(v.y), "=f"(v.z), "=f"(v.w)
               : "l"(mc)
               : "memory");
  return v;
}

template <int D>
__global__ void __launch_bounds__(256) reduce_rows_kernel(const SpmmArgs a, const ReduceArgs r) {
  constexpr int LPR = D / 8;
  constexpr int RPW = 32 / LPR;
  constexpr int HALF = D / 2;
  const int lane = threadIdx.x & 31;
  const int grp = lane / LPR;
  const int gl = lane % LPR;
  const int warp0 = (blockIdx.x * blockDim.x + threadIdx.x) >> 5;
  const int nwarps = (gridDim.x * blockDim.x) >> 5;
  const int n_items = (r.n_slice + RPW - 1) / RPW;
  peer_wait(a.ps);
  if (r.mc_part) {
    constexpr int UN = 4;
    for (int item = warp0 * UN; item < n_items; item += nwarps * UN) {
      float4 p0[UN], p1[UN];
      bool ok[UN];
#pragma unroll
      for (int u = 0; u < UN; ++u) {
        const int k = (item + u) * RPW + grp;
        ok[u] = (item + u) < n_items && k < r.n_slice;
        if (ok[u] && r.mask) {
          const int row = r.slice_begin + k;
          ok[u] = (__ldg(r.mask + (row >> 5)) >> (row & 31)) & 1u;
        }
        p0[u] = p1[u] = f4_zero();
        if (ok[u]) {
          const float* src = r.mc_part + (size_t)(r.slice_begin + k) * D + gl * 4;
          p0[u] = multimem_ld_reduce_add4(src);
          p1[u] = multimem_ld_reduce_add4(src + HALF);
        }
      }
#pragma unroll
      for (int u = 0; u < UN; ++u) {
        if (!__any_sync(SRB_FULL_MASK, ok[u])) continue;
        spmm_epilogue<D>(a, r.slice_begin + (item + u) * RPW + grp, gl, p0[u], p1[u], ok[u]);
      }
    }
    peer_signal(a.ps);
    return;
  }
  for (int item = warp0; item < n_items; item += nwarps) {
    const int k = item * RPW + grp;
    bool valid = k < r.n_slice;
    if (r.mask) {
      const int row = r.slice_begin + k;
      valid = valid && ((__ldg(r.mask + (row >> 5)) >> (row & 31)) & 1u);
      if (!__any_sync(SRB_FULL_MASK, valid)) continue;
    }
    float4 acc0 = f4_zero(), acc1 = f4_zero();
    if (valid) {
      const float* src = r.stage + (size_t)k * D + gl * 4;
      const size_t plane = (size_t)r.stage_cap * D;
#pragma unroll 1
      for (int q = 0; q < r.world; q += 2) {
        const bool two = q + 1 < r.world;
        const float4 p0 = ldg4(src + (size_t)q * plane), p1 = ldg4(src + (size_t)q * plane + HALF);
        float4 p2 = f4_zero(), p3 = f4_zero();
        if (two) {
          p2 = ldg4(src + (size_t)(q + 1) * plane);
          p3 = ldg4(src + (size_t)(q + 1) * plane + HALF);
        }
        acc0 = f4_add(acc0, p0);
        acc1 = f4_add(acc1, p1);
        if (two) {
          acc0 = f4_add(acc0, p2);
          acc1 = f4_add(acc1, p3);
        }
      }
    }
    spmm_epilogue<D>(a, r.slice_begin + k, gl, acc0, acc1, valid);
  }
  peer_signal(a.ps);
}

template <int D>
__global__ void __launch_bounds__(256) rows_epilogue_kernel(const SpmmArgs a) {
  constexpr int LPR = D / 8;
  constexpr int RPW = 32 / LPR;
  constexpr int HALF = D / 2;
  const int lane = threadIdx.x & 31;
  const int grp = lane / LPR;
  const int gl = lane % LPR;
  const int warp0 = (blockIdx.x * blockDim.x + threadIdx.x) >> 5;
  const int nwarps = (gridDim.x * blockDim.x) >> 5;
  const int n_items = (a.n_rows + RPW - 1) / RPW;
  for (int item = warp0; item < n_items; item += nwarps) {
    const int row = item * RPW + grp;
    const bool valid = row < a.n_rows;
    float4 acc0 = f4_zero(), acc1 = f4_zero();
    if (valid) {
      const float* src = a.X + (size_t)row * D + gl * 4;
      acc0 = a.stream ? __ldcs(reinterpret_cast<const float4*>(src)) : ldg4(src);
      acc1 = a.stream ? __ldcs(reinterpret_cast<const float4*>(src + HALF)) : ldg4(src + HALF);
    }
    spmm_epilogue<D>(a, row, gl, acc0, acc1, valid);
  }
}

int launch_rows_epilogue(const SpmmArgs& a, int d, cudaStream_t st) {
  if (a.n_rows <= 0) return SRB_OK;
  const int rpw = 32 / (d / 8);
  long long blocks = ((long long)(a.n_rows + rpw - 1) / rpw + 7) / 8;
  const long long cap = (long long)sm_count() * 8;
  if (blocks > cap) blocks = cap;
  if (blocks < 1) blocks = 1;
  switch (d) {
    case 32: rows_epilogue_kernel<32><<<(int)blocks, 256, 0, st>>>(a); break;
    case 64: rows_epilogue_kernel<64><<<(int)blocks, 256, 0, st>>>(a); break;
    case 128: rows_epilogue_kernel<128><<<(int)blocks, 256, 0, st>>>(a); break;
    default: set_error("rows_epilogue: unsupported d=%d (32, 64, 128)", d); return SRB_ERR_ARG;
  }
  return post_launch("rows_epilogue_kernel");
}

int launch_reduce_rows(const SpmmArgs& a, const ReduceArgs& r, int d, cudaStream_t st) {
  if (r.n_slice <= 0) return SRB_OK;
  const int rpw = 32 / (d / 8);
  long long blocks = ((long long)(r.n_slice + rpw - 1) / rpw + 7) / 8;
  const long long cap = (long long)sm_count() * (r.small_grid ? 1 : 8);
  if (blocks > cap) blocks = cap;
  if (blocks < 1) blocks = 1;
  switch (d) {
    case 32: reduce_rows_kernel<32><<<(int)blocks, 256, 0, st>>>(a, r); break;
    case 64: reduce_rows_kernel<64><<<(int)blocks, 256, 0, st>>>(a, r); break;
    case 128: reduce_rows_kernel<128><<<(int)blocks, 256, 0, st>>>(a, r); break;
    default: set_error("reduce_rows: unsupported d=%d (32, 64, 128)", d); return SRB_ERR_ARG;
  }
  return post_launch("reduce_rows_kernel");
}

template <int D, bool M, bool AS>
static void launch_spmm_dma(const SpmmArgs& a, int hub_blocks, int blocks, cudaStream_t st) {
  if (hub_blocks > 0) {
    if (a.seg && a.n_warp > 0) {
      const int wb = max(1, min((a.n_warp + 7) / 8, blocks));
      spmm_seg_warp_kernel<D, M, AS><<<wb, 256, 0, st>>>(a);
      g_launches.fetch_add(1, std::memory_order_relaxed);
    }
    spmm_hub_kernel<D, M, AS><<<hub_blocks, 256, 0, st>>>(a);
    const int nh = a.n_vlong_dev ? a.n_rows : a.n_huge;
    spmm_hub_finish_kernel<D><<<max(1, min((nh + 7) / 8, hub_blocks)), 256, 0, st>>>(a);
    g_launches.fetch_add(2, std::memory_order_relaxed);
  }
  spmm_csr_kernel<D, M, AS><<<blocks, 256, 0, st>>>(a);
}

template <int D>
static void launch_spmm_d(const SpmmArgs& a, int hub_blocks, int blocks, cudaStream_t st) {
  if (a.col_mask != nullptr) launch_spmm_dma<D, true, false>(a, hub_blocks, blocks, st);
  else if (D >= 64 && a.async_stage) launch_spmm_dma<D, false, (D >= 64)>(a, hub_blocks, blocks, st);
  else launch_spmm_dma<D, false, false>(a, hub_blocks, blocks, st);
}

int launch_spmm(const SpmmArgs& a, int d, cudaStream_t st) {
  if (a.n_rows == 0) return SRB_OK;
  const int threads = 256;
  const int rpw = 32 / (d / 8);
  const long long items = (long long)a.n_long + ((long long)a.n_rows - a.n_huge - a.n_vlong - a.n_long + rpw - 1) / rpw;
  long long blocks = (items + threads / 32 - 1) / (threads / 32);
  if (a.n_vlong_dev) blocks = ((long long)a.n_rows + threads / 32 - 1) / (threads / 32);
  if (blocks < a.n_vlong) blocks = a.n_vlong;
  const long long cap = (long long)sm_count() * 8;
  if (blocks > cap) blocks = cap;
  if (blocks < 1) blocks = 1;
  long long hub_blocks = a.seg ? (a.n_cta > 0 ? a.n_cta : (a.n_work > 0 ? 1 : 0)) : a.n_work;
  if (hub_blocks > cap) hub_blocks = cap;
  switch (d) {
    case 32: launch_spmm_d<32>(a, (int)hub_blocks, (int)blocks, st); break;
    case 64: launch_spmm_d<64>(a, (int)hub_blocks, (int)blocks, st); break;
    case 128: launch_spmm_d<128>(a, (int)hub_blocks, (int)blocks, st); break;
    default: set_error("spmm: unsupported d=%d (32, 64, 128)", d); return SRB_ERR_ARG;
  }
  return post_launch("spmm_csr_kernel");
}

static bool async_stage_enabled() {
  static const int on = [] {
    const char* e = getenv("SRB_SPMM_ASYNC");
    return (e && e[0] == '1') ? 1 : 0;
  }();
  return on != 0;
}

int fill_args(const srb_spmm_desc* d, SpmmArgs& a) {
  SRB_REQUIRE(d != nullptr, "spmm: null desc");
  SRB_REQUIRE(d->rowptr && d->colidx && d->vals && d->X, "spmm: null CSR/X pointer");
  SRB_REQUIRE(d->n_rows >= 0 && d->n_cols >= 0, "spmm: negative shape");
  SRB_REQUIRE(d->noise_mode >= 0 && d->noise_mode <= 2, "spmm: bad noise_mode");
  SRB_REQUIRE(d->noise_mode != 1 || d->noise, "spmm: noise_mode 1 needs a noise tensor");
  SRB_REQUIRE(!d->adam_p || (d->adam_m && d->adam_v && d->adam_scalars), "spmm: incomplete adam pointers");
  SRB_REQUIRE(d->X != d->Y, "spmm: Y must not alias X");
  a.rowptr = d->rowptr;
  a.colidx = d->colidx;
  a.vals = d->vals;
  a.row_order = d->row_order;
  a.n_rows = d->n_rows;
  a.n_vlong_dev = d->row_order ? d->n_vlong_dev : nullptr;
  const bool hub = d->row_order && d->hub.n_work > 0 && (a.n_vlong_dev || d->hub.n_rows > 0);
  SRB_REQUIRE(!hub || (d->hub.first && (d->hub.work || d->hub.seg) && d->hub.part), "spmm: split-row lists incomplete");
  SRB_REQUIRE(!hub || d->hub.n_rows <= d->n_rows, "spmm: more split rows than rows");
  a.n_huge = (hub && !a.n_vlong_dev) ? d->hub.n_rows : 0;
  a.hub_first = hub ? d->hub.first : nullptr;
  a.hub_work = hub ? d->hub.work : nullptr;
  a.hub_part = hub ? d->hub.part : nullptr;
  a.n_work = hub ? d->hub.n_work : 0;
  const bool segs = hub && !a.n_vlong_dev && d->hub.seg != nullptr;
  SRB_REQUIRE(!segs || (d->hub.seg_cnt && (d->hub.n_cta == 0 || d->hub.order_cta) && (d->hub.n_warp == 0 || d->hub.order_warp)),
              "spmm: column-blocked split-row lists incomplete");
  a.seg = segs ? d->hub.seg : nullptr;
  a.seg_cnt = segs ? d->hub.seg_cnt : nullptr;
  a.order_cta = segs ? d->hub.order_cta : nullptr;
  a.order_warp = segs ? d->hub.order_warp : nullptr;
  a.n_cta = segs ? d->hub.n_cta : 0;
  a.n_warp = segs ? d->hub.n_warp : 0;
  const int rest = d->n_rows - a.n_huge;
  a.n_vlong = (d->row_order && d->n_vlong_rows > 0) ? (d->n_vlong_rows < rest ? d->n_vlong_rows : rest) : 0;
  a.col_mask = d->col_mask;
  a.n_long = (d->row_order && d->n_long_rows > 0) ? (d->n_long_rows < rest - a.n_vlong ? d->n_long_rows : rest - a.n_vlong) : 0;
  a.X = d->X;
  a.Y = d->Y;
  a.extra = d->extra;
  a.extra_scale = d->extra_scale;
  a.noise_mode = d->noise_mode;
  a.noise = d->noise;
  a.eps = d->eps;
  a.pkey = make_uint2((uint32_t)d->philox_seed, (uint32_t)(d->philox_seed >> 32));
  a.poff = make_uint2((uint32_t)d->philox_offset, (uint32_t)(d->philox_offset >> 32));
  a.pstep = d->philox_step_dev;
  a.sum_in = d->sum_in;
  a.sum_out = d->sum_out;
  a.sum_scale = d->sum_scale;
  a.ap = d->adam_p;
  a.am = d->adam_m;
  a.av = d->adam_v;
  a.ascal = d->adam_scalars;
  a.b2 = (float)d->beta2;
  a.w1 = (float)(1.0 - d->beta1);
  a.w2 = (float)(1.0 - d->beta2);
  a.aeps = d->adam_eps;
  a.world = 0;
  a.row_begin = 0;
  a.noise_row_base = 0;
  a.noise_row_stride = 1;
  a.peer_mc = 0;
  a.ps = PeerSync{};
  a.stream = ((long long)d->n_rows + d->n_cols) * d->d * 4 > l2_bytes() / 4 * 3;
  a.async_stage = a.stream && async_stage_enabled();
  a.stage_rank = a.stage_cap = 0;
  for (int g = 0; g < 8; ++g) a.peer[g] = a.peer_sum[g] = a.peer_p[g] = a.stage_peer[g] = nullptr;
  for (int g = 0; g < 9; ++g) a.stage_bounds[g] = 0;
  return SRB_OK;
}

}

extern "C" int srb_spmm_csr(const srb_spmm_desc* desc, void* stream) {
  srb::SpmmArgs a;
  SRB_TRY(srb::fill_args(desc, a));
  return srb::launch_spmm(a, desc->d, (cudaStream_t)stream);
}

extern "C" int srb_spmm_epilogue_rows(const srb_spmm_desc* desc, void* stream) {
  srb::SpmmArgs a;
  SRB_TRY(srb::fill_args(desc, a));
  SRB_REQUIRE(desc->Y || desc->sum_out || desc->adam_p, "spmm_epilogue_rows: nothing to write");
  return srb::launch_rows_epilogue(a, desc->d, (cudaStream_t)stream);
}

extern "C" int srb_encoder_forward(const srb_encoder_desc* e, void* stream) {
  SRB_REQUIRE(e != nullptr, "encoder: null desc");
  SRB_REQUIRE(e->E0 && e->final_out, "encoder: null E0/final_out");
  SRB_REQUIRE(e->n_layers >= 0, "encoder: negative n_layers");
  SRB_REQUIRE(e->n_layers == 0 || (e->work0 && e->work1), "encoder: work buffers required");
  SRB_REQUIRE(e->include_ego || e->n_layers > 0, "encoder: mean over zero layers");
  SRB_REQUIRE(!e->last_rows || (e->last_rows_out && e->last_rows_out != e->final_out && e->last_rows_out != e->E0),
              "encoder: last_rows needs a separate last_rows_out buffer");
  const size_t nd = (size_t)e->n * e->d;
  cudaStream_t st = (cudaStream_t)stream;
  const int L = e->n_layers;
  if (L == 0) {
    SRB_TRY(srb::check_cuda(cudaMemcpyAsync(e->final_out, e->E0, nd * 4, cudaMemcpyDeviceToDevice, st), "encoder copy"));
    if (e->cl_out)
      SRB_TRY(srb::check_cuda(cudaMemcpyAsync(e->cl_out, e->E0, nd * 4, cudaMemcpyDeviceToDevice, st), "encoder copy"));
    return SRB_OK;
  }
  const float inv = 1.0f / (float)(e->include_ego ? L + 1 : L);
  const bool want_cl = e->cl_out != nullptr;
  const bool cl_hit = want_cl && e->layer_cl >= 1 && e->layer_cl <= L;
  if (want_cl && !cl_hit)
    SRB_TRY(srb::check_cuda(cudaMemcpyAsync(e->cl_out, e->E0, nd * 4, cudaMemcpyDeviceToDevice, st), "encoder copy"));
  const float* x = e->E0;
  int k0 = 0;
  if (e->x1) {
    SRB_REQUIRE(L >= 2 && !e->include_ego && !(cl_hit && e->layer_cl == 1) && e->x1 != e->work0 && e->x1 != e->work1,
                "encoder: x1 needs n_layers >= 2, include_ego == 0, layer_cl != 1 and a buffer of its own");
    x = e->x1;
    k0 = 1;
  }
  for (int k = k0; k < L; ++k) {
    srb_spmm_desc s = {};
    s.rowptr = e->rowptr;
    s.colidx = e->colidx;
    s.vals = e->vals;
    s.row_order = e->row_order;
    s.n_long_rows = e->n_long_rows;
    s.n_vlong_rows = e->n_vlong_rows;
    s.hub = e->hub;
    s.n_rows = e->n;
    s.n_cols = e->n;
    s.d = e->d;
    s.X = x;
    const bool last = (k == L - 1);
    float* y = nullptr;
    if (cl_hit && k == e->layer_cl - 1) y = e->cl_out;
    else if (!last) y = (x == e->work0) ? e->work1 : e->work0;
    s.Y = y;
    s.noise_mode = e->noise_mode;
    if (e->noise_mode == 1) s.noise = e->noise + (size_t)k * nd;
    s.eps = e->eps;
    s.philox_seed = e->philox_seed;
    s.philox_offset = e->philox_offset + (uint64_t)k;
    s.philox_step_dev = e->philox_step_dev;
    s.sum_in = (k == 0) ? (e->include_ego ? e->E0 : nullptr) : ((k == 1 && e->x1) ? e->x1 : e->final_out);
    s.sum_out = e->final_out;
    s.sum_scale = last ? inv : 1.0f;
    if (last && e->last_rows && e->n_last_rows > 0 && !(cl_hit && k == e->layer_cl - 1)) {
      s.row_order = e->last_rows;
      s.n_rows = e->n_last_rows;
      if (e->last_rows_nv_dev) {
        s.n_vlong_rows = 0;
        s.n_long_rows = 0;
        s.n_vlong_dev = e->last_rows_nv_dev;
        s.hub = e->last_rows_hub;
      } else {
        s.n_vlong_rows = e->n_last_rows;
        s.n_long_rows = 0;
        s.hub = srb_hub_split{};
      }
      s.Y = nullptr;
      s.sum_out = e->last_rows_out;
    }
    SRB_TRY(srb_spmm_csr(&s, stream));
    x = y;
  }
  return SRB_OK;
}
```

selfrec_b200/csrc/spmm_args.cuh:

```cuda
#pragma once
#include "common.cuh"

namespace srb {

struct PeerSync {
  int* flags[8];
  int* epoch;
  int* counter;
  int* err;
  int world, rank;
  int wait, signal;
};

__device__ __forceinline__ void st_release_sys(int* p, int v) { asm volatile("st.release.sys.global.s32 [%0], %1;" ::"l"(p), "r"(v) : "memory"); }
__device__ __forceinline__ int ld_acquire_sys(const int* p) {
  int v;
  asm volatile("ld.acquire.sys.global.s32 %0, [%1];" : "=r"(v) : "l"(p) : "memory");
  return v;
}

__device__ __forceinline__ int ld_relaxed_sys(const int* p) {
  int v;
  asm volatile("ld.relaxed.sys.global.s32 %0, [%1];" : "=r"(v) : "l"(p) : "memory");
  return v;
}

__device__ __forceinline__ void peer_wait(const PeerSync& s) {
  if (!s.wait) return;
  if ((int)threadIdx.x < s.world) {
    const int target = *reinterpret_cast<volatile int*>(s.epoch);
    const int* f = s.flags[s.rank] + threadIdx.x;
    const long long t0 = clock64();
    while (ld_relaxed_sys(f) < target) {
      if (clock64() - t0 > 60000000000ll) {
        *s.err = 1;
        break;
      }
      __nanosleep(20);
    }
    (void)ld_acquire_sys(f);
  }
  __syncthreads();
}

__device__ __forceinline__ void peer_signal(const PeerSync& s) {
  if (!s.signal) return;
  __syncthreads();
  if (threadIdx.x == 0) {
    __threadfence();
    if (atomicAdd(s.counter, 1) == (int)gridDim.x - 1) {
      *s.counter = 0;
      __threadfence_system();
      const int e = *s.epoch + 1;
      *s.epoch = e;
      for (int q = 0; q < s.world; ++q) st_release_sys(s.flags[q] + s.rank, e);
    }
  }
}

struct SpmmArgs {
  const int32_t* rowptr;
  const int32_t* colidx;
  const float* vals;
  const int32_t* row_order;
  int32_t n_rows;
  const int32_t* n_vlong_dev;
  const uint32_t* col_mask;
  int32_t n_huge;
  int32_t n_vlong;
  int32_t n_long;
  const int32_t* hub_first;
  const int32_t* hub_work;
  int32_t n_work;
  float* hub_part;
  const int32_t* seg;
  const int32_t* seg_cnt;
  const int32_t* order_cta;
  const int32_t* order_warp;
  int32_t n_cta;
  int32_t n_warp;
  const float* X;
  float* Y;
  const float* extra;
  float extra_scale;
  int32_t noise_mode;
  const float* noise;
  float eps;
  uint2 pkey;
  uint2 poff;
  const int32_t* pstep;
  const float* sum_in;
  float* sum_out;
  float sum_scale;
  float* ap;
  float* am;
  float* av;
  const float* ascal;
  float b2, w1, w2, aeps;
  int32_t world;
  int32_t row_begin;
  float* peer[8];
  float* peer_sum[8];
  float* peer_p[8];
  int32_t stream;
  int32_t async_stage;
  int32_t peer_mc;
  int32_t noise_row_base;
  int32_t noise_row_stride;
  float* stage_peer[8];
  int32_t stage_bounds[9];
  int32_t stage_rank;
  int32_t stage_cap;
  PeerSync ps;
};

struct ReduceArgs {
  const float* stage;
  int32_t world;
  int32_t stage_cap;
  int32_t slice_begin;
  int32_t n_slice;
  const uint32_t* mask;
  const float* mc_part;
  int32_t small_grid;
};

int launch_spmm(const SpmmArgs& a, int d, cudaStream_t st);
int launch_reduce_rows(const SpmmArgs& a, const ReduceArgs& r, int d, cudaStream_t st);
int launch_rows_epilogue(const SpmmArgs& a, int d, cudaStream_t st);
int fill_args(const srb_spmm_desc* d, SpmmArgs& a);



}
```

Measured before the change: 1768.

## Add programmatic dependent launch, fused step-begin kernel, seeded backward chain, batch-only mean

Routes kernel launches through a cudaLaunchKernelEx helper that sets programmatic stream serialization, and adds griddepcontrol wait/trigger to kernels so launch latency can overlap with the previous kernel. The adam prepare step, the row-mask memset and the zeroing of seed rows are merged into one step_begin kernel. For LightGCN and XSimGCL, the backward chain now scatters gradients into seed buffers that the SpMM kernels read under a row mask, instead of running the old chain. The forward pass computes the final layer mean only on the batch rows by passing extra sum sources. These changes add complexity, and because each kernel triggers its dependents right after its wait, correctness relies on that wait ordering.

```diff
diff --git a/selfrec_b200/csrc/bpr.cu b/selfrec_b200/csrc/bpr.cu
--- a/selfrec_b200/csrc/bpr.cu
+++ b/selfrec_b200/csrc/bpr.cu
@@ -37,6 +37,8 @@
   const int lane = threadIdx.x & 31;
   const int wib = threadIdx.x >> 5;
   const int t = blockIdx.x * (blockDim.x >> 5) + wib;
+  pdl_wait();
+  pdl_trigger();
   const int b = a.b_dev ? min(*a.b_dev, a.b) : a.b;
   float bpr = 0.f, su = 0.f, sp = 0.f, sn = 0.f;
   if (t < b) {
@@ -91,6 +93,8 @@
   constexpr int Q = (D + 127) / 128;
   const int lane = threadIdx.x & 31;
   const int t = blockIdx.x * (blockDim.x >> 5) + (threadIdx.x >> 5);
+  pdl_wait();
+  pdl_trigger();
   const int b = a.b_dev ? min(*a.b_dev, a.b) : a.b;
   const float fb = (float)b;
   const float nu = sqrtf(a.scratch[1]), np = sqrtf(a.scratch[2]), nn = sqrtf(a.scratch[3]);
@@ -160,6 +164,8 @@
   const ScatterSeg& sg = segs.s[blockIdx.y];
   const int lane = threadIdx.x & 31;
   const int r = blockIdx.x * (blockDim.x >> 5) + (threadIdx.x >> 5);
+  pdl_wait();
+  pdl_trigger();
   const int nn = sg.n_dev ? min(*sg.n_dev, sg.n) : sg.n;
   if (r >= nn) return;
   int row = sg.rows[r] + sg.row_off;
@@ -183,12 +189,11 @@
   if (max_n == 0) return SRB_OK;
   dim3 grid((max_n + 7) / 8, segs.count);
   switch (d) {
-    case 32: scatter_add_rows_kernel<32><<<grid, 256, 0, st>>>(dst, segs); break;
-    case 64: scatter_add_rows_kernel<64><<<grid, 256, 0, st>>>(dst, segs); break;
-    case 128: scatter_add_rows_kernel<128><<<grid, 256, 0, st>>>(dst, segs); break;
+    case 32: return launch_kernel(scatter_add_rows_kernel<32>, grid, 256, 0, st, "scatter_add_rows_kernel", dst, segs);
+    case 64: return launch_kernel(scatter_add_rows_kernel<64>, grid, 256, 0, st, "scatter_add_rows_kernel", dst, segs);
+    case 128: return launch_kernel(scatter_add_rows_kernel<128>, grid, 256, 0, st, "scatter_add_rows_kernel", dst, segs);
     default: set_error("scatter: unsupported d=%d (32, 64, 128)", d); return SRB_ERR_ARG;
   }
-  return post_launch("scatter_add_rows_kernel");
 }
 
 struct L2Args {
@@ -234,17 +239,14 @@
 }
 
 __global__ void adam_prepare_kernel(int32_t* step, float* scalars, double lr, double b1, double b2) {
-  const int t = *step + 1;
-  *step = t;
-  const double bc1 = 1.0 - pow(b1, (double)t);
-  const double bc2 = 1.0 - pow(b2, (double)t);
-  scalars[0] = (float)(lr / bc1);
-  scalars[1] = (float)sqrt(bc2);
+  adam_prepare(step, scalars, lr, b1, b2);
 }
 
 __global__ void __launch_bounds__(256) adam_step_kernel(float* __restrict__ p, float* __restrict__ m, float* __restrict__ v,
                                                         const float* __restrict__ g, long long n4, long long n,
                                                         const float* __restrict__ scal, float w1, float b2, float w2, float eps) {
+  pdl_wait();
+  pdl_trigger();
   const float step_size = scal[0], bc2_sqrt = scal[1];
   const long long stride = (long long)gridDim.x * blockDim.x;
   for (long long i = (long long)blockIdx.x * blockDim.x + threadIdx.x; i < n4; i += stride) {
@@ -304,12 +306,10 @@
   SRB_TRY(srb::check_cuda(cudaMemsetAsync(d->scratch, 0, 8 * sizeof(float), st), "bpr memset"));
   const int blocks = d->b > 0 ? (d->b + 7) / 8 : 1;
   switch (d->d) {
-#define SRB_CASE(DD)                                               \
-  case DD:                                                         \
-    srb::bpr_reduce_kernel<DD><<<blocks, 256, 0, st>>>(a);         \
-    SRB_TRY(srb::post_launch("bpr_reduce_kernel"));                \
-    srb::bpr_grad_kernel<DD><<<blocks, 256, 0, st>>>(a);           \
-    return srb::post_launch("bpr_grad_kernel");
+#define SRB_CASE(DD)                                                                                 \
+  case DD:                                                                                           \
+    SRB_TRY(srb::launch_kernel(srb::bpr_reduce_kernel<DD>, blocks, 256, 0, st, "bpr_reduce_kernel", a)); \
+    return srb::launch_kernel(srb::bpr_grad_kernel<DD>, blocks, 256, 0, st, "bpr_grad_kernel", a);
     SRB_CASE(32)
     SRB_CASE(64)
     SRB_CASE(128)
@@ -356,9 +356,8 @@
   const long long cap = (long long)srb::sm_count() * 8;
   if (blocks > cap) blocks = cap;
   if (blocks < 1) blocks = 1;
-  srb::adam_step_kernel<<<(int)blocks, 256, 0, (cudaStream_t)stream>>>(p, m, v, g, n4, n, scalars_dev, (float)(1.0 - beta1), (float)beta2,
-                                                                        (float)(1.0 - beta2), eps);
-  return srb::post_launch("adam_step_kernel");
+  return srb::launch_kernel(srb::adam_step_kernel, (int)blocks, 256, 0, (cudaStream_t)stream, "adam_step_kernel", p, m, v, g, n4, n,
+                            scalars_dev, (float)(1.0 - beta1), (float)beta2, (float)(1.0 - beta2), eps);
 }
 
 extern "C" int srb_l2_reg_fwd(int32_t n_terms, const float* const* x, const int64_t* n_elems, const int32_t* rows, float reg,
diff --git a/selfrec_b200/csrc/common.cuh b/selfrec_b200/csrc/common.cuh
--- a/selfrec_b200/csrc/common.cuh
+++ b/selfrec_b200/csrc/common.cuh
@@ -3,6 +3,7 @@
 #include <stdint.h>
 #include <stdio.h>
 #include <atomic>
+#include <utility>
 #include "selfrec_b200.h"
 
 #define SRB_FULL_MASK 0xffffffffu
@@ -23,6 +24,29 @@
 inline int post_launch(const char* what) {
   g_launches.fetch_add(1, std::memory_order_relaxed);
   return check_cuda(cudaPeekAtLastError(), what);
+}
+
+__device__ __forceinline__ void pdl_wait() { asm volatile("griddepcontrol.wait;" ::: "memory"); }
+__device__ __forceinline__ void pdl_trigger() { asm volatile("griddepcontrol.launch_dependents;" ::: "memory"); }
+
+bool pdl_active();
+
+template <typename... KArgs, typename... Args>
+inline int launch_kernel(void (*kernel)(KArgs...), dim3 grid, dim3 block, size_t smem, cudaStream_t st, const char* what,
+                         Args&&... args) {
+  cudaLaunchAttribute attr[1];
+  attr[0].id = cudaLaunchAttributeProgrammaticStreamSerialization;
+  attr[0].val.programmaticStreamSerializationAllowed = 1;
+  cudaLaunchConfig_t cfg = {};
+  cfg.gridDim = grid;
+  cfg.blockDim = block;
+  cfg.dynamicSmemBytes = smem;
+  cfg.stream = st;
+  cfg.attrs = attr;
+  cfg.numAttrs = pdl_active() ? 1 : 0;
+  const cudaError_t e = cudaLaunchKernelEx(&cfg, kernel, std::forward<Args>(args)...);
+  g_launches.fetch_add(1, std::memory_order_relaxed);
+  return check_cuda(e, what);
 }
 
 #define SRB_REQUIRE(cond, ...)            \
@@ -54,9 +78,18 @@
 };
 struct ScatterSegs {
   int count;
-  ScatterSeg s[8];
+  ScatterSeg s[16];
 };
 int scatter_segments(float* dst, int d, const ScatterSegs& segs, cudaStream_t st);
+
+__device__ __forceinline__ void adam_prepare(int32_t* step, float* scalars, double lr, double b1, double b2) {
+  const int t = *step + 1;
+  *step = t;
+  const double bc1 = 1.0 - pow(b1, (double)t);
+  const double bc2 = 1.0 - pow(b2, (double)t);
+  scalars[0] = (float)(lr / bc1);
+  scalars[1] = (float)sqrt(bc2);
+}
 
 __device__ __forceinline__ float warp_sum(float v) {
 #pragma unroll
diff --git a/selfrec_b200/csrc/engine.cu b/selfrec_b200/csrc/engine.cu
--- a/selfrec_b200/csrc/engine.cu
+++ b/selfrec_b200/csrc/engine.cu
@@ -1,7 +1,25 @@
+#include <stdlib.h>
+#include <algorithm>
 #include <mutex>
-#include "common.cuh"
+#include "spmm_args.cuh"
 
 namespace srb {
+
+static bool pdl_enabled() {
+  static const bool on = [] {
+    const char* e = getenv("SRB_PDL");
+    return !(e && e[0] == '0');
+  }();
+  return on;
+}
+
+static thread_local bool t_pdl = false;
+bool pdl_active() { return t_pdl; }
+
+struct PdlScope {
+  PdlScope() { t_pdl = pdl_enabled(); }
+  ~PdlScope() { t_pdl = false; }
+};
 
 struct Ws {
   float* final_;
@@ -13,6 +31,7 @@
   float* acc1;
   float* gd;
   float* rsum;
+  float* seed;
   float* g_emb;
   float* g_l2;
   float* g_nce;
@@ -33,6 +52,8 @@
 };
 
 static int64_t al(int64_t x) { return (x + 255) / 256 * 256; }
+
+static bool seeded_chain(int model) { return model == SRB_MODEL_LIGHTGCN || model == SRB_MODEL_XSIMGCL; }
 
 static int64_t carve(const srb_step_desc* s, Ws* w, char* base) {
   const int64_t N = (int64_t)s->n_users + s->n_items, d = s->d, B = s->batch_cap;
@@ -55,6 +76,7 @@
   float* f_a1 = (float*)take(graph ? nd : 0);
   float* f_gd = (float*)take(graph ? nd : 0);
   float* f_rsum = (float*)take(graph ? nd : 0);
+  float* f_seed = (float*)take(seeded_chain(s->model) ? 2 * nd : 0);
   float* f_gemb = (float*)take(3 * B * d * 4);
   float* f_gl2 = (float*)take(3 * B * d * 4);
   float* f_gnce = (float*)take(has_cl ? 4 * 2 * B * d * 4 : 0);
@@ -82,6 +104,7 @@
     w->acc1 = f_a1;
     w->gd = f_gd;
     w->rsum = f_rsum;
+    w->seed = seeded_chain(s->model) ? f_seed : nullptr;
     w->g_emb = f_gemb;
     w->g_l2 = f_gl2;
     w->g_nce = f_gnce;
@@ -104,6 +127,8 @@
 }
 
 __global__ void build_cat_idx_kernel(const int32_t* batch, int cap, int n_users, int32_t* idx_cat, int32_t* n_cat) {
+  pdl_wait();
+  pdl_trigger();
   const int nu = min(batch[1], cap), ni = min(batch[2], cap);
   const int32_t* uu = batch + SRB_BATCH_HEADER + 3 * cap;
   const int32_t* ui = uu + cap;
@@ -117,6 +142,8 @@
                                                                uint32_t* row_mask, int32_t* hub_first, int32_t* hub_work,
                                                                int hub_cap) {
   const int t = blockIdx.x * blockDim.x + threadIdx.x;
+  pdl_wait();
+  pdl_trigger();
   const int b = min(batch[0], cap);
   const int sec = t / cap, k = t % cap;
   if (sec >= 3 || k >= b) return;
@@ -147,7 +174,28 @@
   }
 }
 
+__global__ void __launch_bounds__(256) step_begin_kernel(int32_t* step, float* scalars, double lr, double b1, double b2, int32_t* words,
+                                                         int n_words, const int32_t* batch, int cap, int n_users, int n, int d,
+                                                         float* seed) {
+  pdl_wait();
+  pdl_trigger();
+  const int t = blockIdx.x * blockDim.x + threadIdx.x;
+  if (t == 0) adam_prepare(step, scalars, lr, b1, b2);
+  if (t < n_words) words[t] = 0;
+  if (!seed) return;
+  const int per_row = d / 4;
+  const int r = t / per_row, c = (t % per_row) * 4;
+  const int sec = r / cap, k = r % cap;
+  if (sec >= 3 || k >= min(batch[0], cap)) return;
+  const int32_t* u = batch + SRB_BATCH_HEADER;
+  const size_t row = (sec == 0) ? u[k] : n_users + u[sec * cap + k];
+  st4(seed + row * d + c, f4_zero());
+  st4(seed + ((size_t)n + row) * d + c, f4_zero());
+}
+
 __global__ void finalize_losses_kernel(const float* bpr_losses, const float* nce_losses, int n_nce, float cl_rate, float* out) {
+  pdl_wait();
+  pdl_trigger();
   float cl = 0.f;
   for (int q = 0; q < n_nce; ++q) cl += nce_losses[q];
   cl *= cl_rate;
@@ -167,7 +215,8 @@
 };
 
 static int spmm_simple(const srb_step_desc* s, const srb_graph_csr* g, const float* x, float* y, const float* extra,
-                       bool adam, cudaStream_t st, const uint32_t* col_mask = nullptr) {
+                       bool adam, cudaStream_t st, const uint32_t* col_mask = nullptr, const float* seed = nullptr,
+                       const uint32_t* seed_mask = nullptr) {
   srb_spmm_desc p = {};
   p.col_mask = col_mask;
   p.rowptr = g->rowptr;
@@ -192,7 +241,11 @@
     p.beta2 = s->beta2;
     p.adam_eps = s->adam_eps;
   }
-  return srb_spmm_csr(&p, st);
+  SpmmArgs a;
+  SRB_TRY(fill_args(&p, a));
+  a.seed_mask = seed_mask;
+  a.seed = seed;
+  return launch_spmm(a, p.d, st);
 }
 
 struct ForkRes {
@@ -226,7 +279,7 @@
 static ScatterSegs merged(const ScatterSegs& a, const ScatterSegs* b) {
   ScatterSegs m = a;
   if (b)
-    for (int q = 0; q < b->count && m.count < 8; ++q) m.s[m.count++] = b->s[q];
+    for (int q = 0; q < b->count && m.count < 16; ++q) m.s[m.count++] = b->s[q];
   return m;
 }
 
@@ -257,6 +310,29 @@
   SRB_TRY(spmm_simple(s, c.adj, x, w.gd, extra, false, st, mask));
   *gd_live = true;
   return SRB_OK;
+}
+
+static int run_chain_seeded(const srb_step_desc* s, const Ws& w, const Chain& c, cudaStream_t st) {
+  const int L = s->n_layers, d = s->d, N = s->n_users + s->n_items;
+  float* F = w.seed;
+  float* G = w.seed + (size_t)N * d;
+  const ScatterSegs* cs = c.layer_cl >= 1 ? &c.cl_segs : (c.ego_segs.count ? &c.ego_segs : nullptr);
+  const int c_level = cs == &c.cl_segs ? c.layer_cl : (cs ? 0 : -1);
+  ScatterSegs sg = c.final_segs;
+  if (cs) {
+    ScatterSegs sc = (c_level >= 1 || c.include_ego) ? merged(c.final_segs, cs) : *cs;
+    for (int q = 0; q < sc.count; ++q) sc.s[q].row_off += N;
+    sg = merged(sg, &sc);
+  }
+  SRB_TRY(scatter_segments(F, d, sg, st));
+  const float* x = c_level == L ? G : F;
+  for (int k = L - 1; k >= 1; --k) {
+    float* y = (x == w.acc0) ? w.acc1 : w.acc0;
+    SRB_TRY(spmm_simple(s, c.adj, x, y, nullptr, false, st, k == L - 1 ? w.row_mask : nullptr, c_level == k ? G : F, w.row_mask));
+    x = y;
+  }
+  const float* seed0 = c_level == 0 ? G : (c.include_ego ? F : nullptr);
+  return spmm_simple(s, c.adj, x, nullptr, nullptr, true, st, L == 1 ? w.row_mask : nullptr, seed0, w.row_mask);
 }
 
 static ScatterSeg seg(const float* src, const int32_t* rows, const int32_t* n_dev, int n, int row_off, float scale) {
@@ -365,13 +441,17 @@
   const int32_t* nu_dev = hdr + 1;
   const int32_t* ni_dev = hdr + 2;
 
-  SRB_TRY(srb_adam_prepare(s->step_dev, s->scalars, s->lr, s->beta1, s->beta2, stream));
+  PdlScope pdl;
 
   if (s->model != SRB_MODEL_MF) {
-    SRB_TRY(check_cuda(cudaMemsetAsync(w.n_hub, 0, 32 + (size_t)((U + s->n_items + 31) / 32) * 4, st), "row mask memset"));
-    build_batch_rows_kernel<<<(3 * B + 255) / 256, 256, 0, st>>>(s->batch, B, U, s->adj.rowptr, 0, U + s->n_items, w.batch_rows, w.n_hub,
-                                                                   w.row_mask, w.hub_cap ? w.hub_first : nullptr, w.hub_work, w.hub_cap);
-    SRB_TRY(post_launch("build_batch_rows_kernel"));
+    const int n_words = 8 + (U + s->n_items + 31) / 32;
+    const int threads = w.seed ? std::max(n_words, 3 * B * (d / 4)) : n_words;
+    SRB_TRY(launch_kernel(step_begin_kernel, (threads + 255) / 256, 256, 0, st, "step_begin_kernel", s->step_dev, s->scalars, s->lr,
+                          s->beta1, s->beta2, w.n_hub, n_words, s->batch, B, U, N, d, w.seed));
+    SRB_TRY(launch_kernel(build_batch_rows_kernel, (3 * B + 255) / 256, 256, 0, st, "build_batch_rows_kernel", s->batch, B, U, s->adj.rowptr, 0,
+                          U + s->n_items, w.batch_rows, w.n_hub, w.row_mask, w.hub_cap ? w.hub_first : nullptr, w.hub_work, w.hub_cap));
+  } else {
+    SRB_TRY(srb_adam_prepare(s->step_dev, s->scalars, s->lr, s->beta1, s->beta2, stream));
   }
   const float* table = s->params;
   int n_nce = 0;
@@ -463,8 +543,7 @@
     SRB_TRY(srb_infonce_fwd_bwd(&q, stream));
     n_nce = 2;
   } else if (s->model == SRB_MODEL_SGL) {
-    build_cat_idx_kernel<<<8, 256, 0, st>>>(s->batch, B, U, w.idx_cat, w.n_cat);
-    SRB_TRY(post_launch("build_cat_idx_kernel"));
+    SRB_TRY(launch_kernel(build_cat_idx_kernel, 8, 256, 0, st, "build_cat_idx_kernel", s->batch, B, U, w.idx_cat, w.n_cat));
     srb_infonce_desc q = {};
     q.n_problems = 1;
     q.d = d;
@@ -477,8 +556,8 @@
     n_nce = 1;
   }
   if (fk) SRB_TRY(check_cuda(cudaStreamWaitEvent(st, fk->join, 0), "join wait"));
-  finalize_losses_kernel<<<1, 1, 0, st>>>(w.bpr_losses, w.nce_losses, n_nce, s->cl_rate, s->losses);
-  SRB_TRY(post_launch("finalize_losses_kernel"));
+  SRB_TRY(launch_kernel(finalize_losses_kernel, 1, 1, 0, st, "finalize_losses_kernel", w.bpr_losses, w.nce_losses, n_nce, s->cl_rate,
+                        s->losses));
 
   const size_t plane = (size_t)B * d;
   if (s->model == SRB_MODEL_MF) {
@@ -534,5 +613,5 @@
     f.s[5] = seg(g2a, uq_u, nu_dev, B, 0, cm);
     f.s[6] = seg(g2b, uq_i, ni_dev, B, U, cm);
   }
-  return run_chain(s, w, c, &gd_live, true, st);
-}
+  return seeded_chain(s->model) ? run_chain_seeded(s, w, c, st) : run_chain(s, w, c, &gd_live, true, st);
+}
diff --git a/selfrec_b200/csrc/infonce.cu b/selfrec_b200/csrc/infonce.cu
--- a/selfrec_b200/csrc/infonce.cu
+++ b/selfrec_b200/csrc/infonce.cu
@@ -53,6 +53,8 @@
 
 template <int D>
 __global__ void __launch_bounds__(256) nce_prep_kernel(const NceArgs a) {
+  pdl_wait();
+  pdl_trigger();
   const NceProblem& p = a.p[blockIdx.y];
   const int lane = threadIdx.x & 31;
   const int i = blockIdx.x * (blockDim.x >> 5) + (threadIdx.x >> 5);
@@ -116,6 +118,8 @@
 }
 
 __global__ void __launch_bounds__(256) nce_prep_tc_kernel(const NceArgs a) {
+  pdl_wait();
+  pdl_trigger();
   constexpr int D = 64;
   __shared__ float t1[32][D + 1], t2[32][D + 1];
   const NceProblem& p = a.p[blockIdx.y];
@@ -221,6 +225,8 @@
 
 template <int D>
 __global__ void __launch_bounds__(256) nce_lse_kernel(const NceArgs a) {
+  pdl_wait();
+  pdl_trigger();
   extern __shared__ __align__(16) unsigned char smem_raw[];
   NceLseSmem<D>& sm = *reinterpret_cast<NceLseSmem<D>*>(smem_raw);
   const NceProblem& p = a.p[blockIdx.z];
@@ -294,6 +300,8 @@
 
 template <int D>
 __global__ void __launch_bounds__(256) nce_grad_kernel(const NceArgs a) {
+  pdl_wait();
+  pdl_trigger();
   constexpr int CW = D / 16;
   extern __shared__ __align__(16) unsigned char smem_raw[];
   NceGradSmem<D>& sm = *reinterpret_cast<NceGradSmem<D>*>(smem_raw);
@@ -411,6 +419,8 @@
 
 template <int D>
 __global__ void __launch_bounds__(256) nce_finish_kernel(const NceArgs a) {
+  pdl_wait();
+  pdl_trigger();
   const NceProblem& p = a.p[blockIdx.y];
   const int lane = threadIdx.x & 31;
   const int i = blockIdx.x * (blockDim.x >> 5) + (threadIdx.x >> 5);
@@ -456,6 +466,8 @@
 }
 
 __global__ void __launch_bounds__(256) nce_tc_finish_kernel(const NceArgs a) {
+  pdl_wait();
+  pdl_trigger();
   constexpr int D = 64;
   const NceProblem& p = a.p[blockIdx.y];
   const int lane = threadIdx.x & 31;
@@ -499,8 +511,7 @@
   const int d = NT_D;
   {
     dim3 grid(np / 32, n_problems);
-    nce_prep_tc_kernel<<<grid, 256, 0, st>>>(a);
-    SRB_TRY(post_launch("nce_prep_tc_kernel"));
+    SRB_TRY(launch_kernel(nce_prep_tc_kernel, grid, 256, 0, st, "nce_prep_tc_kernel", a));
   }
   NtMaps maps;
   NtArgs t;
@@ -556,16 +567,9 @@
     attr_done = true;
   }
   dim3 grid(row_blocks, splits, n_problems);
-  nce_tc_kernel<1><<<grid, NT_THREADS, smem, st>>>(maps, t);
-  SRB_TRY(post_launch("nce_tc_kernel<pass_a>"));
-  nce_tc_kernel<2><<<grid, NT_THREADS, smem, st>>>(maps, t);
-  SRB_TRY(post_launch("nce_tc_kernel<pass_b>"));
-  {
-    dim3 g2((np + 7) / 8, n_problems);
-    nce_tc_finish_kernel<<<g2, 256, 0, st>>>(a);
-    SRB_TRY(post_launch("nce_tc_finish_kernel"));
-  }
-  return SRB_OK;
+  SRB_TRY(launch_kernel(nce_tc_kernel<1>, grid, NT_THREADS, smem, st, "nce_tc_kernel<pass_a>", maps, t));
+  SRB_TRY(launch_kernel(nce_tc_kernel<2>, grid, NT_THREADS, smem, st, "nce_tc_kernel<pass_b>", maps, t));
+  return launch_kernel(nce_tc_finish_kernel, dim3((np + 7) / 8, n_problems), 256, 0, st, "nce_tc_finish_kernel", a);
 }
 
 template <int D>
@@ -573,8 +577,7 @@
   const int np = a.np;
   {
     dim3 grid((np + 7) / 8, n_problems);
-    nce_prep_kernel<D><<<grid, 256, 0, st>>>(a);
-    SRB_TRY(post_launch("nce_prep_kernel"));
+    SRB_TRY(launch_kernel(nce_prep_kernel<D>, grid, 256, 0, st, "nce_prep_kernel", a));
   }
   {
     static bool attr_done = false;
@@ -584,15 +587,12 @@
       attr_done = true;
     }
     dim3 grid(np / NCE_T, a.splits, n_problems);
-    nce_lse_kernel<D><<<grid, 256, sizeof(NceLseSmem<D>), st>>>(a);
-    SRB_TRY(post_launch("nce_lse_kernel"));
-    nce_grad_kernel<D><<<grid, 256, sizeof(NceGradSmem<D>), st>>>(a);
-    SRB_TRY(post_launch("nce_grad_kernel"));
+    SRB_TRY(launch_kernel(nce_lse_kernel<D>, grid, 256, sizeof(NceLseSmem<D>), st, "nce_lse_kernel", a));
+    SRB_TRY(launch_kernel(nce_grad_kernel<D>, grid, 256, sizeof(NceGradSmem<D>), st, "nce_grad_kernel", a));
   }
   {
     dim3 grid((np + 7) / 8, n_problems);
-    nce_finish_kernel<D><<<grid, 256, 0, st>>>(a);
-    SRB_TRY(post_launch("nce_finish_kernel"));
+    SRB_TRY(launch_kernel(nce_finish_kernel<D>, grid, 256, 0, st, "nce_finish_kernel", a));
   }
   return SRB_OK;
 }
diff --git a/selfrec_b200/csrc/infonce_tc.cuh b/selfrec_b200/csrc/infonce_tc.cuh
--- a/selfrec_b200/csrc/infonce_tc.cuh
+++ b/selfrec_b200/csrc/infonce_tc.cuh
@@ -64,6 +64,8 @@
 
 template <int MODE>
 __global__ void __launch_bounds__(NT_THREADS, 1) nce_tc_kernel(const __grid_constant__ NtMaps maps, const NtArgs a) {
+  pdl_wait();
+  pdl_trigger();
   extern __shared__ __align__(1024) uint8_t nt_smem_raw[];
   uint8_t* sm = reinterpret_cast<uint8_t*>((reinterpret_cast<uintptr_t>(nt_smem_raw) + 1023) & ~(uintptr_t)1023);
   uint64_t* bars = reinterpret_cast<uint64_t*>(sm + NtSmem::bar_off);
diff --git a/selfrec_b200/csrc/spmm.cu b/selfrec_b200/csrc/spmm.cu
--- a/selfrec_b200/csrc/spmm.cu
+++ b/selfrec_b200/csrc/spmm.cu
@@ -34,6 +34,13 @@
       y0 = f4_fma(a.extra_scale, *reinterpret_cast<const float4*>(a.extra + off), y0);
       y1 = f4_fma(a.extra_scale, *reinterpret_cast<const float4*>(a.extra + off + HALF), y1);
     }
+    if (a.seed && valid) {
+      const int grow = a.row_begin + row;
+      if ((__ldg(a.seed_mask + (grow >> 5)) >> (grow & 31)) & 1u) {
+        y0 = f4_add(y0, *reinterpret_cast<const float4*>(a.seed + off));
+        y1 = f4_add(y1, *reinterpret_cast<const float4*>(a.seed + off + HALF));
+      }
+    }
     if (a.noise_mode) {
       float4 n0 = f4_zero(), n1 = f4_zero();
       if (a.noise_mode == 1) {
@@ -74,8 +81,16 @@
     if (a.sum_out) {
       float4 s0 = y0, s1 = y1;
       if (a.sum_in) {
-        s0 = f4_add(s0, *reinterpret_cast<const float4*>(a.sum_in + off));
-        s1 = f4_add(s1, *reinterpret_cast<const float4*>(a.sum_in + off + HALF));
+        float4 t0 = *reinterpret_cast<const float4*>(a.sum_in + off);
+        float4 t1 = *reinterpret_cast<const float4*>(a.sum_in + off + HALF);
+#pragma unroll
+        for (int j = 0; j < 3; ++j) {
+          if (!a.sum_add[j]) break;
+          t0 = f4_add(*reinterpret_cast<const float4*>(a.sum_add[j] + off), t0);
+          t1 = f4_add(*reinterpret_cast<const float4*>(a.sum_add[j] + off + HALF), t1);
+        }
+        s0 = f4_add(s0, t0);
+        s1 = f4_add(s1, t1);
       }
       s0 = f4_scale(a.sum_scale, s0);
       s1 = f4_scale(a.sum_scale, s1);
@@ -262,6 +277,8 @@
   float4* stg = ASYNC ? stage + wib * SPMM_STAGE_F4 + lane : nullptr;
   const int grp = lane / LPR;
   const int gl = lane % LPR;
+  pdl_wait();
+  pdl_trigger();
   const int n_work = a.seg ? a.n_cta : (a.n_vlong_dev ? min(a.n_vlong_dev[4], a.n_work) : a.n_work);
   __shared__ float4 part[8][2][LPR];
   for (int k = blockIdx.x; k < n_work; k += gridDim.x) {
@@ -314,6 +331,8 @@
   const int gl = lane % LPR;
   const int warp0 = (blockIdx.x * blockDim.x + threadIdx.x) >> 5;
   const int nwarps = (gridDim.x * blockDim.x) >> 5;
+  pdl_wait();
+  pdl_trigger();
   for (int k = warp0; k < a.n_warp; k += nwarps) {
     const int w = __ldg(a.order_warp + k);
     const int beg = __ldg(a.seg + 2 * w), end = __ldg(a.seg + 2 * w + 1);
@@ -337,6 +356,8 @@
   const int gl = lane % LPR;
   const int warp0 = (blockIdx.x * blockDim.x + threadIdx.x) >> 5;
   const int nwarps = (gridDim.x * blockDim.x) >> 5;
+  pdl_wait();
+  pdl_trigger();
   const int n_huge = a.n_vlong_dev ? min(a.n_vlong_dev[0], a.n_rows) : a.n_huge;
   peer_wait(a.ps);
   for (int vr = warp0; vr < n_huge; vr += nwarps) {
@@ -368,6 +389,8 @@
   const int warp0 = (blockIdx.x * blockDim.x + threadIdx.x) >> 5;
   const int nwarps = (gridDim.x * blockDim.x) >> 5;
 
+  pdl_wait();
+  pdl_trigger();
   peer_wait(a.ps);
   int n_vlong = a.n_vlong, n_long = a.n_long, n_short = a.n_rows - a.n_huge - a.n_vlong - a.n_long;
   const int32_t* ro_v = a.row_order ? a.row_order + a.n_huge : nullptr;
@@ -530,6 +553,8 @@
   const int warp0 = (blockIdx.x * blockDim.x + threadIdx.x) >> 5;
   const int nwarps = (gridDim.x * blockDim.x) >> 5;
   const int n_items = (a.n_rows + RPW - 1) / RPW;
+  pdl_wait();
+  pdl_trigger();
   for (int item = warp0; item < n_items; item += nwarps) {
     const int row = item * RPW + grp;
     const bool valid = row < a.n_rows;
@@ -551,12 +576,11 @@
   if (blocks > cap) blocks = cap;
   if (blocks < 1) blocks = 1;
   switch (d) {
-    case 32: rows_epilogue_kernel<32><<<(int)blocks, 256, 0, st>>>(a); break;
-    case 64: rows_epilogue_kernel<64><<<(int)blocks, 256, 0, st>>>(a); break;
-    case 128: rows_epilogue_kernel<128><<<(int)blocks, 256, 0, st>>>(a); break;
+    case 32: return launch_kernel(rows_epilogue_kernel<32>, (int)blocks, 256, 0, st, "rows_epilogue_kernel", a);
+    case 64: return launch_kernel(rows_epilogue_kernel<64>, (int)blocks, 256, 0, st, "rows_epilogue_kernel", a);
+    case 128: return launch_kernel(rows_epilogue_kernel<128>, (int)blocks, 256, 0, st, "rows_epilogue_kernel", a);
     default: set_error("rows_epilogue: unsupported d=%d (32, 64, 128)", d); return SRB_ERR_ARG;
   }
-  return post_launch("rows_epilogue_kernel");
 }
 
 int launch_reduce_rows(const SpmmArgs& a, const ReduceArgs& r, int d, cudaStream_t st) {
@@ -576,26 +600,24 @@
 }
 
 template <int D, bool M, bool AS>
-static void launch_spmm_dma(const SpmmArgs& a, int hub_blocks, int blocks, cudaStream_t st) {
+static int launch_spmm_dma(const SpmmArgs& a, int hub_blocks, int blocks, cudaStream_t st) {
   if (hub_blocks > 0) {
     if (a.seg && a.n_warp > 0) {
       const int wb = max(1, min((a.n_warp + 7) / 8, blocks));
-      spmm_seg_warp_kernel<D, M, AS><<<wb, 256, 0, st>>>(a);
-      g_launches.fetch_add(1, std::memory_order_relaxed);
-    }
-    spmm_hub_kernel<D, M, AS><<<hub_blocks, 256, 0, st>>>(a);
+      SRB_TRY(launch_kernel(spmm_seg_warp_kernel<D, M, AS>, wb, 256, 0, st, "spmm_seg_warp_kernel", a));
+    }
+    SRB_TRY(launch_kernel(spmm_hub_kernel<D, M, AS>, hub_blocks, 256, 0, st, "spmm_hub_kernel", a));
     const int nh = a.n_vlong_dev ? a.n_rows : a.n_huge;
-    spmm_hub_finish_kernel<D><<<max(1, min((nh + 7) / 8, hub_blocks)), 256, 0, st>>>(a);
-    g_launches.fetch_add(2, std::memory_order_relaxed);
-  }
-  spmm_csr_kernel<D, M, AS><<<blocks, 256, 0, st>>>(a);
+    SRB_TRY(launch_kernel(spmm_hub_finish_kernel<D>, max(1, min((nh + 7) / 8, hub_blocks)), 256, 0, st, "spmm_hub_finish_kernel", a));
+  }
+  return launch_kernel(spmm_csr_kernel<D, M, AS>, blocks, 256, 0, st, "spmm_csr_kernel", a);
 }
 
 template <int D>
-static void launch_spmm_d(const SpmmArgs& a, int hub_blocks, int blocks, cudaStream_t st) {
-  if (a.col_mask != nullptr) launch_spmm_dma<D, true, false>(a, hub_blocks, blocks, st);
-  else if (D >= 64 && a.async_stage) launch_spmm_dma<D, false, (D >= 64)>(a, hub_blocks, blocks, st);
-  else launch_spmm_dma<D, false, false>(a, hub_blocks, blocks, st);
+static int launch_spmm_d(const SpmmArgs& a, int hub_blocks, int blocks, cudaStream_t st) {
+  if (a.col_mask != nullptr) return launch_spmm_dma<D, true, false>(a, hub_blocks, blocks, st);
+  if (D >= 64 && a.async_stage) return launch_spmm_dma<D, false, (D >= 64)>(a, hub_blocks, blocks, st);
+  return launch_spmm_dma<D, false, false>(a, hub_blocks, blocks, st);
 }
 
 int launch_spmm(const SpmmArgs& a, int d, cudaStream_t st) {
@@ -612,12 +634,11 @@
   long long hub_blocks = a.seg ? (a.n_cta > 0 ? a.n_cta : (a.n_work > 0 ? 1 : 0)) : a.n_work;
   if (hub_blocks > cap) hub_blocks = cap;
   switch (d) {
-    case 32: launch_spmm_d<32>(a, (int)hub_blocks, (int)blocks, st); break;
-    case 64: launch_spmm_d<64>(a, (int)hub_blocks, (int)blocks, st); break;
-    case 128: launch_spmm_d<128>(a, (int)hub_blocks, (int)blocks, st); break;
+    case 32: return launch_spmm_d<32>(a, (int)hub_blocks, (int)blocks, st);
+    case 64: return launch_spmm_d<64>(a, (int)hub_blocks, (int)blocks, st);
+    case 128: return launch_spmm_d<128>(a, (int)hub_blocks, (int)blocks, st);
     default: set_error("spmm: unsupported d=%d (32, 64, 128)", d); return SRB_ERR_ARG;
   }
-  return post_launch("spmm_csr_kernel");
 }
 
 static bool async_stage_enabled() {
@@ -667,6 +688,8 @@
   a.Y = d->Y;
   a.extra = d->extra;
   a.extra_scale = d->extra_scale;
+  a.seed_mask = nullptr;
+  a.seed = nullptr;
   a.noise_mode = d->noise_mode;
   a.noise = d->noise;
   a.eps = d->eps;
@@ -674,6 +697,7 @@
   a.poff = make_uint2((uint32_t)d->philox_offset, (uint32_t)(d->philox_offset >> 32));
   a.pstep = d->philox_step_dev;
   a.sum_in = d->sum_in;
+  a.sum_add[0] = a.sum_add[1] = a.sum_add[2] = nullptr;
   a.sum_out = d->sum_out;
   a.sum_scale = d->sum_scale;
   a.ap = d->adam_p;
@@ -743,6 +767,20 @@
     x = e->x1;
     k0 = 1;
   }
+  const bool last_on_rows = e->last_rows && e->n_last_rows > 0 && !(cl_hit && e->layer_cl == L);
+  const float* src[4];
+  int n_src = 0;
+  bool live = true;
+  if (e->include_ego) src[n_src++] = e->E0;
+  const float* px = e->E0;
+  for (int k = 0; k < L - 1 && live; ++k) {
+    const float* py = (k == 0 && e->x1) ? e->x1 : (cl_hit && k == e->layer_cl - 1) ? e->cl_out : (px == e->work0 ? e->work1 : e->work0);
+    for (int j = 0; j < n_src; ++j) live = live && src[j] != py;
+    live = live && n_src < 4;
+    if (live) src[n_src++] = py;
+    px = py;
+  }
+  const bool batch_mean = last_on_rows && live;
   for (int k = k0; k < L; ++k) {
     srb_spmm_desc s = {};
     s.rowptr = e->rowptr;
@@ -768,9 +806,10 @@
     s.philox_offset = e->philox_offset + (uint64_t)k;
     s.philox_step_dev = e->philox_step_dev;
     s.sum_in = (k == 0) ? (e->include_ego ? e->E0 : nullptr) : ((k == 1 && e->x1) ? e->x1 : e->final_out);
-    s.sum_out = e->final_out;
+    s.sum_out = (batch_mean && !last) ? nullptr : e->final_out;
     s.sum_scale = last ? inv : 1.0f;
-    if (last && e->last_rows && e->n_last_rows > 0 && !(cl_hit && k == e->layer_cl - 1)) {
+    if (batch_mean && last) s.sum_in = n_src ? src[0] : nullptr;
+    if (last && last_on_rows) {
       s.row_order = e->last_rows;
       s.n_rows = e->n_last_rows;
       if (e->last_rows_nv_dev) {
@@ -786,7 +825,11 @@
       s.Y = nullptr;
       s.sum_out = e->last_rows_out;
     }
-    SRB_TRY(srb_spmm_csr(&s, stream));
+    srb::SpmmArgs a;
+    SRB_TRY(srb::fill_args(&s, a));
+    if (batch_mean && last)
+      for (int j = 1; j < n_src; ++j) a.sum_add[j - 1] = src[j];
+    SRB_TRY(srb::launch_spmm(a, s.d, st));
     x = y;
   }
   return SRB_OK;
diff --git a/selfrec_b200/csrc/spmm_args.cuh b/selfrec_b200/csrc/spmm_args.cuh
--- a/selfrec_b200/csrc/spmm_args.cuh
+++ b/selfrec_b200/csrc/spmm_args.cuh
@@ -83,6 +83,8 @@
   float* Y;
   const float* extra;
   float extra_scale;
+  const uint32_t* seed_mask;
+  const float* seed;
   int32_t noise_mode;
   const float* noise;
   float eps;
@@ -90,6 +92,7 @@
   uint2 poff;
   const int32_t* pstep;
   const float* sum_in;
+  const float* sum_add[3];
   float* sum_out;
   float sum_scale;
   float* ap;
```

Measured after the change: 1910 (median of 6 runs). 8.0% higher.
